# pengfeidip/pytorch-faster-rcnn

Measured on NVIDIA B200. Metric: images/sec of RPN proposal+assign+RoIAlign, R50-FPN 800x1333, higher is better.
Workload: dtype f32

## Files before the change

include/b200det.h:

```cpp
#ifndef B200DET_H_
#define B200DET_H_

#include <stddef.h>
#include <stdint.h>

#ifdef __cplusplus
extern "C" {
#endif

#if defined(__GNUC__)
#define B2D_API __attribute__((visibility("default")))
#else
#define B2D_API
#endif

#define B2D_OK 0
#define B2D_ERR_ARG (-1)
#define B2D_MAX_LEVELS 8
#define B2D_MAX_ANCHORS 16

typedef struct b2d_level {
    int H, W, A;
    int center_lt;
    float stride;
    float ws[B2D_MAX_ANCHORS], hs[B2D_MAX_ANCHORS];
    long long offset;
} b2d_level;

typedef struct b2d_pyramid {
    int num_levels;
    int _pad;
    long long total;
    b2d_level lv[B2D_MAX_LEVELS];
} b2d_pyramid;

B2D_API const char* b2d_last_error_string(void);
B2D_API int b2d_version(void);
B2D_API void b2d_reload_knobs(void);

B2D_API int b2d_anchor_grid(float* out, const float* ws, const float* hs, int A, int H, int W, float stride,
                    int center_lt, void* stream);
B2D_API int b2d_inside_anchor_mask(uint8_t* mask, const float* anchors, long long n, float img_h, float img_w,
                           float border, void* stream);
B2D_API int b2d_inside_grid_mask(float* flags, int A, int H, int W, int in_h, int in_w, void* stream);

B2D_API int b2d_calc_iou(float* out , const float* a , long long N, const float* b ,
                 long long K, void* stream);
B2D_API int b2d_elem_iou(float* out , const float* a, const float* b, long long N, void* stream);

B2D_API int b2d_assign_max_iou(int64_t* labels, float* max_iou, long long out_ld, const float* boxes,
                       long long box_ld, const int* box_count, long long N, const b2d_pyramid* pyr_host,
                       const float* img_hw, float border, const float* gt, int gt_ld, const int* gt_count,
                       int B, float pos_iou, float neg_iou, float min_pos_iou, int prepend_gt, int* census,
                       int* pos_list, int pos_cap, void* workspace, size_t ws_bytes, void* stream);

B2D_API int b2d_sample_labels(int* chosen, int* n_chosen, const int64_t* labels, long long ld, const int* count,
                      const int* count_add , long long n, const int* census, const int* pos_list, int pos_cap, int B, int max_num,
                      int pos_num, unsigned long long seed, const unsigned long long* seed_step , void* stream);
B2D_API int b2d_counter_add(unsigned long long* cell, unsigned long long inc, void* stream);
B2D_API int b2d_label_census(int* census, int* pos_list, int pos_cap, const int64_t* labels, long long ld,
                     const int* count, long long n, int B, void* stream);
B2D_API int b2d_scatter_sampled(int64_t* out, const int64_t* labels, long long ld, long long n, const int* chosen,
                        const int* n_chosen, int max_num, int B, void* stream);

B2D_API int b2d_bbox2param(float* out, const float* base, const float* bbox, long long n, const float* means_host,
                   const float* stds_host, void* stream);
B2D_API int b2d_param2bbox(float* out, const float* base, const float* param, long long n, const float* means_host,
                   const float* stds_host, int clamp, float img_h, float img_w, void* stream);
B2D_API int b2d_clamp_bbox(float* out, const float* bbox, long long n, float img_h, float img_w, void* stream);

B2D_API int b2d_encode_targets(float* tar_box, float* tar_gt, float* tar_param, int64_t* tar_label, int64_t* tar_is_gt,
                       const int* chosen, const int* n_chosen, int max_num, const int64_t* labels,
                       long long label_ld, const float* boxes, long long box_ld, const b2d_pyramid* pyr_host,
                       const float* gt, int gt_ld, const int* gt_count, const int64_t* gt_label,
                       int prepend_gt, const float* means_host, const float* stds_host, int B, void* stream);

B2D_API int b2d_roi_targets_fused(int64_t* labels, float* max_iou, long long out_ld, const float* boxes, long long box_ld,
                          const int* box_count, long long N, const float* gt, int gt_ld, const int* gt_count,
                          const int64_t* gt_label, int B, float pos_iou, float neg_iou, float min_pos_iou,
                          int prepend_gt, int* census, int* pos_list, int pos_cap, int* chosen, int* n_chosen,
                          int max_num, int pos_num, unsigned long long seed, const unsigned long long* seed_step,
                          float* tar_box, float* tar_gt, float* tar_param, int64_t* tar_label, int64_t* tar_is_gt,
                          const float* means_host, const float* stds_host, void* stream);

B2D_API int b2d_gather_head_outputs(float* tar_cls, float* tar_reg, const void* const* cls_ptrs_host,
                            const void* const* reg_ptrs_host, const b2d_pyramid* pyr_host, int cls_channels,
                            const int* chosen, const int* n_chosen, int max_num, int B, void* stream);

typedef struct b2d_rpn_cfg {
    int pre_nms, post_nms, max_num;
    int score_mode, num_cls_channels;
    float nms_thr_f;
    float min_size;
    float means[4], stds[4];
    int do_nms;
    float* records;
    void* event_after_select;
} b2d_rpn_cfg;

typedef struct b2d_roi_target_args {
    int64_t* labels; float* max_iou; long long out_ld;
    const float* gt; int gt_ld; const int* gt_count; const int64_t* gt_label;
    float pos_iou, neg_iou, min_pos_iou; int prepend_gt;
    int* census; int* pos_list; int pos_cap;
    int* chosen; int* n_chosen; int max_num, pos_num;
    unsigned long long seed; const unsigned long long* seed_step;
    float* tar_box; float* tar_gt; float* tar_param; int64_t* tar_label; int64_t* tar_is_gt;
    float means[4], stds[4];
} b2d_roi_target_args;

B2D_API size_t b2d_rpn_proposals_workspace_bytes(const b2d_pyramid* pyr_host, int B, const b2d_rpn_cfg* cfg_host);
B2D_API int b2d_last_launch_count(void);
B2D_API size_t b2d_rpn_proposals_debug_offset(const b2d_pyramid* pyr_host, int B, const b2d_rpn_cfg* cfg_host);
B2D_API int b2d_rpn_proposals(float* props, float* scores, int* count, int* prov, const void* const* cls_ptrs_host,
                      const void* const* reg_ptrs_host, const b2d_pyramid* pyr_host, const float* img_hw,
                      int B, const b2d_rpn_cfg* cfg_host, void* workspace, size_t ws_bytes, void* stream);

B2D_API int b2d_rpn_proposals_targets(float* props, float* scores, int* count, int* prov, const void* const* cls_ptrs_host,
                              const void* const* reg_ptrs_host, const b2d_pyramid* pyr_host, const float* img_hw,
                              int B, const b2d_rpn_cfg* cfg_host, void* workspace, size_t ws_bytes,
                              const b2d_roi_target_args* tg_host, void* stream);

B2D_API size_t b2d_topk_workspace_bytes(long long n_max, int S, int k);
B2D_API int b2d_topk(int* idx, int* out_count, const float* values, long long ld, const int* counts, long long n,
             int S, int k, void* workspace, size_t ws_bytes, void* stream);

B2D_API size_t b2d_nms_workspace_bytes(long long n_max, int S);
B2D_API int b2d_nms(int64_t* keep, int* keep_count, const float* boxes, const float* scores, long long n_ld,
            const int* counts, long long n, int S, float thr_f, int max_keep, int presorted, void* workspace,
            size_t ws_bytes, void* stream);

B2D_API size_t b2d_multiclass_nms_workspace_bytes(int cap);
B2D_API int b2d_multiclass_nms(float* out_box, float* out_score, int64_t* out_label, int* out_count, const float* bbox,
                       int box_classes, const float* score, long long n, int C, const unsigned long long* chan_mask_host,
                       float min_score, const float* score_factor, int strict, float nms_thr_f, int max_keep, int cap,
                       int* overflow, void* workspace, size_t ws_bytes, void* stream);
B2D_API int b2d_multiclass_candidates(float* cand_box, float* nms_box, float* cand_score, int* cand_label, int* cand_count,
                              int* overflow, const float* bbox, int box_classes, const float* score, long long n, int C,
                              const unsigned long long* chan_mask_host, float min_score, const float* score_factor,
                              int strict, int cap, void* stream);
B2D_API int b2d_batched_nms_boxes(float* out, const float* bbox, const int64_t* label, long long n, void* stream);
B2D_API int b2d_ga_pack_scores(float* out, long long ld, const void* const* cls_ptrs_host, const void* const* mask_ptrs_host,
                       const int* n_host, int L, void* stream);
B2D_API int b2d_ga_decode(float* box, float* score, int* nvalid, const int* idx, const float* packed, long long ld, int k,
                  const void* const* cls_ptrs_host, const void* const* mask_ptrs_host, const void* const* anchor_ptrs_host,
                  const void* const* reg_ptrs_host, const int* n_host, int L, const float* means_host, const float* stds_host,
                  float img_h, float img_w, float min_size, void* stream);
B2D_API int b2d_scale_rois(float* out, const float* rois, long long ld, long long n, float scale, void* stream);
B2D_API int b2d_iou_bin_ids(int* ids, const int64_t* labels, const float* iou, long long n, int num_bins,
                    const float* bin_lo_host, const float* bin_hi_host, void* stream);
B2D_API int b2d_sample_iou_balanced(int64_t* out_labels, const int64_t* labels, const float* iou, long long n, int max_num,
                            int pos_num, int num_bins, const float* bin_lo_host, const float* bin_hi_host,
                            unsigned long long seed, void* stream);
B2D_API size_t b2d_sampled_ce_workspace_bytes(void);
B2D_API int b2d_sampled_ce_fwd(float* partial, const float* logits, long long ld, int C, int row_major, int sigmoid,
                       const int64_t* target, long long rows, void* stream);
B2D_API int b2d_sampled_ce_bwd(float* grad, const float* scale, const float* logits, long long ld, int C, int row_major,
                       int sigmoid, const int64_t* target, long long rows, void* stream);

B2D_API size_t b2d_anchor_loss_workspace_bytes(const b2d_pyramid* pyr_host, int B);
B2D_API int b2d_anchor_loss_fwd(float* out3, const void* const* cls_ptrs_host, const void* const* reg_ptrs_host,
                        const b2d_pyramid* pyr_host, const int64_t* labels, long long label_ld, const float* gt, int gt_ld,
                        const int64_t* gt_label, int cls_channels, float alpha, float gamma, float beta,
                        const float* means_host, const float* stds_host, int B, void* workspace, size_t ws_bytes,
                        void* stream);
B2D_API int b2d_anchor_loss_bwd(void* const* dcls_ptrs_host, void* const* dreg_ptrs_host, const float* scale2,
                        const void* const* cls_ptrs_host, const void* const* reg_ptrs_host, const b2d_pyramid* pyr_host,
                        const int64_t* labels, long long label_ld, const float* gt, int gt_ld, const int64_t* gt_label,
                        int cls_channels, float alpha, float gamma, float beta, const float* means_host,
                        const float* stds_host, int B, void* stream);

B2D_API int b2d_fcos_targets(int64_t* cls_tar, float* reg_tar, float* ctr_tar, const b2d_pyramid* pyr_host, const float* gt,
                     int gt_ld, const int* gt_count, const int64_t* gt_label, const float* img_hw,
                     const float* level_thr_host, int B, void* stream);

B2D_API size_t b2d_rcnn_detect_workspace_bytes(int cap, int B);
B2D_API int b2d_rcnn_detect(float* out_box, float* out_score, int64_t* out_label, int* out_count, const float* props,
                    long long ld, const int* counts, long long n, const float* cls_out, const float* reg_out, int C,
                    int reg_classes, const float* means_host, const float* stds_host, const float* img_hw,
                    float min_score, float nms_thr_f, int max_per_img, int strict, int cap, int B, int* overflow,
                    void* workspace, size_t ws_bytes, void* stream);
B2D_API int b2d_rcnn_detect_records(float* out_box, float* out_score, int64_t* out_label, int* out_count, float* records,
                            const float* props, long long ld, const int* counts, long long n, const float* cls_out,
                            const float* reg_out, int C, int reg_classes, const float* means_host, const float* stds_host,
                            const float* img_hw, float min_score, float nms_thr_f, int max_per_img, int strict, int cap,
                            int B, int* overflow, void* workspace, size_t ws_bytes, void* stream);

typedef struct b2d_dense_levels {
    int num_levels, _pad;
    long long offset[B2D_MAX_LEVELS];
    const float* base[B2D_MAX_LEVELS];
    long long img_stride[B2D_MAX_LEVELS], class_stride[B2D_MAX_LEVELS];
} b2d_dense_levels;
B2D_API int b2d_dense_detect(float* out_box, float* out_score, int64_t* out_label, int* out_count, const float* boxes,
                     long long ld, const int* counts, const int* rows, const b2d_dense_levels* lv_host, int C, int transform,
                     const float* score_factor, long long factor_ld, const unsigned long long* chan_mask_host,
                     float min_score, int label_add, float nms_thr_f, int max_per_img, int strict, int cap, int B,
                     int* overflow, void* workspace, size_t ws_bytes, void* const* events_host, void* stream);
B2D_API int b2d_dense_detect_records(float* out_box, float* out_score, int64_t* out_label, int* out_count, float* records,
                             const float* boxes, long long ld, const int* counts, const int* rows,
                             const b2d_dense_levels* lv_host, int C, int transform, const float* score_factor,
                             long long factor_ld, const unsigned long long* chan_mask_host, float min_score, int label_add,
                             float nms_thr_f, int max_per_img, int strict, int cap, int B, int* overflow, void* workspace,
                             size_t ws_bytes, void* const* events_host, void* stream);

typedef struct b2d_roi_cfg {
    int num_levels, C, PH, PW, sampling_ratio, aligned, layout;
    float finest_scale;
    int H[B2D_MAX_LEVELS], W[B2D_MAX_LEVELS];
    float spatial_scale[B2D_MAX_LEVELS];
} b2d_roi_cfg;

B2D_API int b2d_roi_align_fwd(float* out, const void* const* feat_ptrs_host, const float* rois, long long roi_ld,
                      const int* roi_img, const int* levels, long long R, const b2d_roi_cfg* cfg_host,
                      void* stream);
B2D_API int b2d_roi_align_fwd_batched(float* out, const void* const* feat_ptrs_host, const float* rois, long long ld,
                              const int* counts, int B, const b2d_roi_cfg* cfg_host, void* stream);
B2D_API size_t b2d_roi_align_bwd_workspace_bytes(long long R, int B, const b2d_roi_cfg* cfg_host);
B2D_API int b2d_roi_align_bwd(void* const* grad_feat_ptrs_host, const float* grad_out, const float* rois,
                      long long roi_ld, const int* roi_img, const int* levels, long long R, int B,
                      const b2d_roi_cfg* cfg_host, void* workspace, size_t ws_bytes, void* stream);
B2D_API int b2d_nchw_to_nhwc(float* dst, const float* src, int B, int C, int H, int W, void* stream);
B2D_API int b2d_roi_levels(int* levels, const float* rois, long long roi_ld, long long R, float finest_scale,
                   int num_levels, void* stream);

B2D_API size_t b2d_roi_cell_bitmap_bytes(int B, const b2d_roi_cfg* cfg_host);
B2D_API int b2d_roi_mark_cells(void* bitmap, const float* rois, long long ld, const int* counts, int B,
                       const b2d_roi_cfg* cfg_host, void* stream);
B2D_API int b2d_fetch_marked_cells(void* const* dst_ptrs_host, const void* const* src_ptrs_host, const void* bitmap,
                           int B, const b2d_roi_cfg* cfg_host, unsigned long long* moved_cells, void* stream);

B2D_API int b2d_roi_pool_fwd(float* out, int* argmax, const float* feat, int B, int C, int H, int W, const float* rois,
                     long long roi_ld, const int* roi_img, long long R, float spatial_scale, int PH, int PW,
                     void* stream);
B2D_API int b2d_roi_pool_bwd(float* grad_feat, const float* grad_out, const int* argmax, int B, int C, int H, int W,
                     const float* rois, long long roi_ld, const int* roi_img, long long R, float spatial_scale,
                     int PH, int PW, void* workspace, size_t ws_bytes, void* stream);

B2D_API int b2d_refine_bboxes(float* out, int* out_count, const float* props, long long ld, const int* counts,
                      long long n, const int64_t* label, const float* reg_out, int C, const int64_t* is_gt,
                      const float* means_host, const float* stds_host, int clamp, const float* img_hw, int B,
                      void* stream);
B2D_API int b2d_refine_bboxes_argmax(float* out, int* out_count, const float* props, long long ld, const int* counts,
                             long long n, const float* cls_out, int num_classes, const float* reg_out,
                             int reg_classes, const float* means_host, const float* stds_host, const float* img_hw,
                             int B, void* stream);

B2D_API size_t b2d_atss_workspace_bytes(const b2d_pyramid* pyr_host, int B);
B2D_API int b2d_atss_assign(int64_t* cls_tar, float* reg_tar, float* ctr_tar, const b2d_pyramid* pyr_host,
                    const float* gt, int gt_ld, const int* gt_count, const int64_t* gt_label, const float* img_hw,
                    int B, int topk, void* workspace, size_t ws_bytes, void* stream);

B2D_API int b2d_fcos_decode(float* boxes, float* key, float* score, float* ctr_score, const void* const* cls_ptrs_host,
                    const void* const* reg_ptrs_host, const void* const* ctr_ptrs_host, const b2d_pyramid* pyr_host,
                    int cls_channels, float reg_mean, float reg_std, float min_size, const float* img_hw, int B,
                    void* stream);
B2D_API size_t b2d_dense_select_workspace_bytes(const int* level_sizes_host, int num_levels, int B, int pre_nms);
B2D_API int b2d_dense_select(int* idx, int* count, float* sel_boxes, const float* key, const float* boxes,
                     const int* level_sizes_host, int num_levels, int B, int pre_nms, void* workspace, size_t ws_bytes,
                     void* stream);

#ifdef __cplusplus
}
#endif
#endif
```

pytorch-faster-rcnn_b200/_C.py:

```python
import ctypes
import os

import numpy as np
import torch

_HERE = os.path.dirname(os.path.abspath(__file__))
LIB_PATH = os.path.join(_HERE, "libb200det.so")

MAX_LEVELS = 8
MAX_ANCHORS = 16

c_void_p, c_int, c_ll, c_float, c_size_t, c_ull = (ctypes.c_void_p, ctypes.c_int, ctypes.c_longlong,
                                                   ctypes.c_float, ctypes.c_size_t, ctypes.c_ulonglong)


class Level(ctypes.Structure):
    _fields_ = [("H", c_int), ("W", c_int), ("A", c_int), ("center_lt", c_int), ("stride", c_float),
                ("ws", c_float * MAX_ANCHORS), ("hs", c_float * MAX_ANCHORS), ("offset", c_ll)]


class Pyramid(ctypes.Structure):
    _fields_ = [("num_levels", c_int), ("_pad", c_int), ("total", c_ll), ("lv", Level * MAX_LEVELS)]


class RpnCfg(ctypes.Structure):
    _fields_ = [("pre_nms", c_int), ("post_nms", c_int), ("max_num", c_int), ("score_mode", c_int),
                ("num_cls_channels", c_int), ("nms_thr_f", c_float), ("min_size", c_float),
                ("means", c_float * 4), ("stds", c_float * 4), ("do_nms", c_int), ("records", c_void_p), ("event_after_select", c_void_p)]


class RoiTargetArgs(ctypes.Structure):
    _fields_ = [("labels", c_void_p), ("max_iou", c_void_p), ("out_ld", c_ll), ("gt", c_void_p), ("gt_ld", c_int),
                ("gt_count", c_void_p), ("gt_label", c_void_p), ("pos_iou", c_float), ("neg_iou", c_float),
                ("min_pos_iou", c_float), ("prepend_gt", c_int), ("census", c_void_p), ("pos_list", c_void_p),
                ("pos_cap", c_int), ("chosen", c_void_p), ("n_chosen", c_void_p), ("max_num", c_int), ("pos_num", c_int),
                ("seed", c_ull), ("seed_step", c_void_p), ("tar_box", c_void_p), ("tar_gt", c_void_p),
                ("tar_param", c_void_p), ("tar_label", c_void_p), ("tar_is_gt", c_void_p), ("means", c_float * 4),
                ("stds", c_float * 4)]


class RoiCfg(ctypes.Structure):
    _fields_ = [("num_levels", c_int), ("C", c_int), ("PH", c_int), ("PW", c_int), ("sampling_ratio", c_int),
                ("aligned", c_int), ("layout", c_int), ("finest_scale", c_float), ("H", c_int * MAX_LEVELS),
                ("W", c_int * MAX_LEVELS), ("spatial_scale", c_float * MAX_LEVELS)]


class DenseLevels(ctypes.Structure):
    _fields_ = [("num_levels", c_int), ("_pad", c_int), ("offset", c_ll * MAX_LEVELS), ("base", c_void_p * MAX_LEVELS),
                ("img_stride", c_ll * MAX_LEVELS), ("class_stride", c_ll * MAX_LEVELS)]


class B200DetError(RuntimeError):
    pass


_lib = None

_P = c_void_p
_SIGS = {
    "b2d_anchor_grid": [_P, _P, _P, c_int, c_int, c_int, c_float, c_int, _P],
    "b2d_inside_anchor_mask": [_P, _P, c_ll, c_float, c_float, c_float, _P],
    "b2d_inside_grid_mask": [_P, c_int, c_int, c_int, c_int, c_int, _P],
    "b2d_calc_iou": [_P, _P, c_ll, _P, c_ll, _P],
    "b2d_elem_iou": [_P, _P, _P, c_ll, _P],
    "b2d_assign_max_iou": [_P, _P, c_ll, _P, c_ll, _P, c_ll, _P, _P, c_float, _P, c_int, _P, c_int, c_float,
                           c_float, c_float, c_int, _P, _P, c_int, _P, c_size_t, _P],
    "b2d_sample_labels": [_P, _P, _P, c_ll, _P, _P, c_ll, _P, _P, c_int, c_int, c_int, c_int, c_ull, _P, _P],
    "b2d_counter_add": [_P, c_ull, _P],
    "b2d_roi_targets_fused": [_P, _P, c_ll, _P, c_ll, _P, c_ll, _P, c_int, _P, _P, c_int, c_float, c_float, c_float,
                              c_int, _P, _P, c_int, _P, _P, c_int, c_int, c_ull, _P, _P, _P, _P, _P, _P, _P, _P, _P],
    "b2d_anchor_loss_fwd": [_P, _P, _P, _P, _P, c_ll, _P, c_int, _P, c_int, c_float, c_float, c_float, _P, _P, c_int, _P,
                            c_size_t, _P],
    "b2d_anchor_loss_bwd": [_P, _P, _P, _P, _P, _P, _P, c_ll, _P, c_int, _P, c_int, c_float, c_float, c_float, _P, _P,
                            c_int, _P],
    "b2d_fcos_targets": [_P, _P, _P, _P, _P, c_int, _P, _P, _P, _P, c_int, _P],
    "b2d_rcnn_detect": [_P, _P, _P, _P, _P, c_ll, _P, c_ll, _P, _P, c_int, c_int, _P, _P, _P, c_float, c_float, c_int,
                        c_int, c_int, c_int, _P, _P, c_size_t, _P],
    "b2d_rcnn_detect_records": [_P, _P, _P, _P, _P, _P, c_ll, _P, c_ll, _P, _P, c_int, c_int, _P, _P, _P, c_float, c_float,
                                c_int, c_int, c_int, c_int, _P, _P, c_size_t, _P],
    "b2d_dense_detect": [_P, _P, _P, _P, _P, c_ll, _P, _P, _P, c_int, c_int, _P, c_ll, _P, c_float, c_int, c_float, c_int,
                         c_int, c_int, c_int, _P, _P, c_size_t, _P, _P],
    "b2d_dense_detect_records": [_P, _P, _P, _P, _P, _P, c_ll, _P, _P, _P, c_int, c_int, _P, c_ll, _P, c_float, c_int, c_float,
                                 c_int, c_int, c_int, c_int, _P, _P, c_size_t, _P, _P],
    "b2d_dense_select": [_P, _P, _P, _P, _P, _P, c_int, c_int, c_int, _P, c_size_t, _P],
    "b2d_gather_head_outputs": [_P, _P, _P, _P, _P, c_int, _P, _P, c_int, c_int, _P],
    "b2d_roi_align_fwd_batched": [_P, _P, _P, c_ll, _P, c_int, _P, _P],
    "b2d_label_census": [_P, _P, c_int, _P, c_ll, _P, c_ll, c_int, _P],
    "b2d_scatter_sampled": [_P, _P, c_ll, c_ll, _P, _P, c_int, c_int, _P],
    "b2d_bbox2param": [_P, _P, _P, c_ll, _P, _P, _P],
    "b2d_param2bbox": [_P, _P, _P, c_ll, _P, _P, c_int, c_float, c_float, _P],
    "b2d_clamp_bbox": [_P, _P, c_ll, c_float, c_float, _P],
    "b2d_encode_targets": [_P, _P, _P, _P, _P, _P, _P, c_int, _P, c_ll, _P, c_ll, _P, _P, c_int, _P, _P, c_int,
                           _P, _P, c_int, _P],
    "b2d_rpn_proposals": [_P, _P, _P, _P, _P, _P, _P, _P, c_int, _P, _P, c_size_t, _P],
    "b2d_rpn_proposals_targets": [_P, _P, _P, _P, _P, _P, _P, _P, c_int, _P, _P, c_size_t, _P, _P],
    "b2d_topk": [_P, _P, _P, c_ll, _P, c_ll, c_int, c_int, _P, c_size_t, _P],
    "b2d_nms": [_P, _P, _P, _P, c_ll, _P, c_ll, c_int, c_float, c_int, c_int, _P, c_size_t, _P],
    "b2d_roi_align_fwd": [_P, _P, _P, c_ll, _P, _P, c_ll, _P, _P],
    "b2d_roi_align_bwd": [_P, _P, _P, c_ll, _P, _P, c_ll, c_int, _P, _P, c_size_t, _P],
    "b2d_roi_levels": [_P, _P, c_ll, c_ll, c_float, c_int, _P],
    "b2d_nchw_to_nhwc": [_P, _P, c_int, c_int, c_int, c_int, _P],
    "b2d_refine_bboxes": [_P, _P, _P, c_ll, _P, c_ll, _P, _P, c_int, _P, _P, _P, c_int, _P, c_int, _P],
    "b2d_refine_bboxes_argmax": [_P, _P, _P, c_ll, _P, c_ll, _P, c_int, _P, c_int, _P, _P, _P, c_int, _P],
    "b2d_atss_assign": [_P, _P, _P, _P, _P, c_int, _P, _P, _P, c_int, c_int, _P, c_size_t, _P],
    "b2d_fcos_decode": [_P, _P, _P, _P, _P, _P, _P, _P, c_int, c_float, c_float, c_float, _P, c_int, _P],
    "b2d_roi_pool_fwd": [_P, _P, _P, c_int, c_int, c_int, c_int, _P, c_ll, _P, c_ll, c_float, c_int, c_int, _P],
    "b2d_multiclass_nms": [_P, _P, _P, _P, _P, c_int, _P, c_ll, c_int, _P, c_float, _P, c_int, c_float, c_int, c_int, _P, _P,
                           c_size_t, _P],
    "b2d_multiclass_candidates": [_P, _P, _P, _P, _P, _P, _P, c_int, _P, c_ll, c_int, _P, c_float, _P, c_int, c_int, _P],
    "b2d_batched_nms_boxes": [_P, _P, _P, c_ll, _P],
    "b2d_scale_rois": [_P, _P, c_ll, c_ll, c_float, _P],
    "b2d_iou_bin_ids": [_P, _P, _P, c_ll, c_int, _P, _P, _P],
    "b2d_sample_iou_balanced": [_P, _P, _P, c_ll, c_int, c_int, c_int, _P, _P, c_ull, _P],
    "b2d_sampled_ce_fwd": [_P, _P, c_ll, c_int, c_int, c_int, _P, c_ll, _P],
    "b2d_sampled_ce_bwd": [_P, _P, _P, c_ll, c_int, c_int, c_int, _P, c_ll, _P],
    "b2d_ga_pack_scores": [_P, c_ll, _P, _P, _P, c_int, _P],
    "b2d_ga_decode": [_P, _P, _P, _P, _P, c_ll, c_int, _P, _P, _P, _P, _P, c_int, _P, _P, c_float, c_float, c_float, _P],
    "b2d_roi_mark_cells": [_P, _P, c_ll, _P, c_int, _P, _P],
    "b2d_fetch_marked_cells": [_P, _P, _P, c_int, _P, _P, _P],
    "b2d_roi_pool_bwd": [_P, _P, _P, c_int, c_int, c_int, c_int, _P, c_ll, _P, c_ll, c_float, c_int, c_int, _P,
                         c_size_t, _P],
}
_SIZE_FNS = {
    "b2d_rpn_proposals_workspace_bytes": [_P, c_int, _P],
    "b2d_rpn_proposals_debug_offset": [_P, c_int, _P],
    "b2d_topk_workspace_bytes": [c_ll, c_int, c_int],
    "b2d_nms_workspace_bytes": [c_ll, c_int],
    "b2d_roi_align_bwd_workspace_bytes": [c_ll, c_int, _P],
    "b2d_atss_workspace_bytes": [_P, c_int],
    "b2d_rcnn_detect_workspace_bytes": [c_int, c_int],
    "b2d_dense_select_workspace_bytes": [_P, c_int, c_int, c_int],
    "b2d_anchor_loss_workspace_bytes": [_P, c_int],
    "b2d_multiclass_nms_workspace_bytes": [c_int],
    "b2d_sampled_ce_workspace_bytes": [],
    "b2d_roi_cell_bitmap_bytes": [c_int, _P],
}
EXPORTS = sorted(list(_SIGS) + list(_SIZE_FNS) + ["b2d_last_error_string", "b2d_version", "b2d_reload_knobs", "b2d_last_launch_count"])


def lib():
    global _lib
    if _lib is not None:
        return _lib
    if not os.path.exists(LIB_PATH):
        raise B200DetError(
            "libb200det.so is not built (%s). Run `python __graft_entry__.py build` "
            "(nvcc, sm_100a). There is no CPU or PyTorch fallback." % LIB_PATH)
    L = ctypes.CDLL(LIB_PATH)
    for name, sig in _SIGS.items():
        fn = getattr(L, name)
        fn.argtypes = sig
        fn.restype = c_int
    for name, sig in _SIZE_FNS.items():
        fn = getattr(L, name)
        fn.argtypes = sig
        fn.restype = c_size_t
    L.b2d_last_error_string.restype = ctypes.c_char_p
    L.b2d_version.restype = c_int
    L.b2d_reload_knobs.restype = None
    L.b2d_last_launch_count.restype = c_int
    _lib = L
    return L


def reload_knobs():
    lib().b2d_reload_knobs()


def check(rc, what):
    if rc != 0:
        msg = lib().b2d_last_error_string().decode("utf-8", "replace")
        raise B200DetError("%s failed (rc=%d): %s" % (what, rc, msg))


def call(name, *args):
    check(getattr(lib(), name)(*args), name)


def ptr(t):
    if t is None:
        return None
    return c_void_p(t.data_ptr())


def stream():
    return c_void_p(torch.cuda.current_stream().cuda_stream)


def require_cuda(*tensors):
    for t in tensors:
        if t is not None and not t.is_cuda:
            raise B200DetError("b200det kernels need CUDA tensors (got a %s tensor); there is no CPU fallback"
                               % t.device.type)


def f32c(t):
    if t.dtype != torch.float32:
        t = t.to(torch.float32)
    return t.contiguous()


def host_f4(v, default):
    a = np.asarray(default if v is None else v, dtype=np.float32).reshape(-1)
    if a.size != 4:
        raise ValueError("expected 4 values, got %r" % (v,))
    return (c_float * 4)(*a.tolist())


def floor_f32(x):
    f = np.float32(x)
    if float(f) > float(x):
        f = np.nextafter(f, np.float32(-np.inf), dtype=np.float32)
    return float(f)


def make_pyramid(levels):
    if not 1 <= len(levels) <= MAX_LEVELS:
        raise ValueError("1..%d levels supported" % MAX_LEVELS)
    p = Pyramid()
    p.num_levels = len(levels)
    off = 0
    for i, lv in enumerate(levels):
        A = len(lv["ws"])
        if not 1 <= A <= MAX_ANCHORS:
            raise ValueError("1..%d anchors per cell supported" % MAX_ANCHORS)
        L = p.lv[i]
        L.H, L.W, L.A = int(lv["H"]), int(lv["W"]), A
        L.center_lt = int(bool(lv.get("center_lt", False)))
        L.stride = float(lv["stride"])
        for a in range(A):
            L.ws[a] = float(lv["ws"][a])
            L.hs[a] = float(lv["hs"][a])
        L.offset = off
        off += A * L.H * L.W
    p.total = off
    return p
```

pytorch-faster-rcnn_b200/csrc/assign.cu:

```cuda
#include <cstdlib>
#include <cstring>

#include "common.cuh"
#include "targets_common.cuh"

namespace b2d {

__device__ __forceinline__ void grid_limits(const b2d_level& lv, float img_h, float img_w, int& in_h, int& in_w) {
    const double r = 1.0 / (double)lv.stride;
    in_h = min(lv.H, (int)((double)img_h * r) + 1);
    in_w = min(lv.W, (int)((double)img_w * r) + 1);
}

__device__ __forceinline__ bool load_box(const AssignArgs& p, const b2d_pyramid& pyr, int b, long long i,
                                         long long n_b, Box& bx, const int* __restrict__ s_lim) {
    if (i >= n_b) return false;
    if (!p.use_pyr) {
        const float* src = p.boxes + (long long)b * 4 * p.box_ld;
        bx.x1 = src[i]; bx.y1 = src[p.box_ld + i]; bx.x2 = src[2 * p.box_ld + i]; bx.y2 = src[3 * p.box_ld + i];
        return true;
    }
    int l = 0;
#pragma unroll
    for (int q = 1; q < kMaxLevels; ++q)
        if (q < pyr.num_levels && i >= pyr.lv[q].offset) l = q;
    const b2d_level& lv = pyr.lv[l];
    const int li = (int)(i - lv.offset);
    const int hw = lv.H * lv.W;
    const int a = li / hw, r = li - a * hw;
    const int y = r / lv.W, x = r - y * lv.W;
    bx = anchor_at(lv, a, y, x);
    const float img_h = p.img_hw[2 * b], img_w = p.img_hw[2 * b + 1];
    bool ok = (y < s_lim[2 * l]) && (x < s_lim[2 * l + 1]);
    if (p.border >= 0.0f)
        ok = ok && bx.x1 >= -p.border && bx.y1 >= -p.border && bx.x2 < img_w + p.border && bx.y2 < img_h + p.border;
    return ok;
}

__global__ void __launch_bounds__(256) k_assign_colmax(AssignArgs p, b2d_pyramid pyr, uint32_t* __restrict__ colmax) {
    __shared__ Box s_gt[kGtChunk];
    __shared__ float s_ga[kGtChunk];
    __shared__ uint32_t s_max[kGtChunk];
    const int b = blockIdx.y;
    const int K = p.gt_count[b];
    const long long n_b = p.box_count ? (long long)p.box_count[b] : p.N;
    const float* g = p.gt + (long long)b * 4 * p.gt_ld;
    const uint32_t kNegInf = f2key(-INFINITY), kZero = f2key(0.0f);
    __shared__ int s_lim[2 * kMaxLevels];
    if (p.use_pyr && threadIdx.x < pyr.num_levels)
        grid_limits(pyr.lv[threadIdx.x], p.img_hw[2 * b], p.img_hw[2 * b + 1], s_lim[2 * threadIdx.x], s_lim[2 * threadIdx.x + 1]);
    __syncthreads();

    Box bx[kBoxesPerThread];
    float ba[kBoxesPerThread];
    bool ok[kBoxesPerThread];
    const long long base = ((long long)blockIdx.x * blockDim.x) * kBoxesPerThread + threadIdx.x;
#pragma unroll
    for (int r = 0; r < kBoxesPerThread; ++r) {
        ok[r] = load_box(p, pyr, b, base + (long long)r * blockDim.x, n_b, bx[r], s_lim);
        ba[r] = ok[r] ? area_plus1(bx[r]) : 0.0f;
    }
    bool any_ok = false;
#pragma unroll
    for (int r = 0; r < kBoxesPerThread; ++r) any_ok |= ok[r];
    any_ok = __any_sync(0xffffffffu, any_ok);
    for (int j0 = 0; j0 < K; j0 += kGtChunk) {
        const int kc = min(kGtChunk, K - j0);
        __syncthreads();
        for (int j = threadIdx.x; j < kc; j += blockDim.x) {
            Box t{g[j0 + j], g[p.gt_ld + j0 + j], g[2 * p.gt_ld + j0 + j], g[3 * p.gt_ld + j0 + j]};
            s_gt[j] = t; s_ga[j] = area_plus1(t); s_max[j] = kNegInf;
        }
        __syncthreads();
        for (int j = 0; j < kc; ++j) {
            const Box t = s_gt[j];
            const float ta = s_ga[j];
            uint32_t m = any_ok ? kZero : kNegInf;
#pragma unroll
            for (int r = 0; r < kBoxesPerThread; ++r) {
                if (!ok[r]) continue;
                const bool hit = fmaxf(bx[r].x1, t.x1) < fminf(bx[r].x2, t.x2) && fmaxf(bx[r].y1, t.y1) < fminf(bx[r].y2, t.y2);
                if (hit || !(ba[r] > 0.0f && ta > 0.0f)) {
                    const float v = iou_plus1(bx[r], ba[r], t, ta) + 0.0f;
                    m = max(m, f2key(v));
                }
            }
            if (__any_sync(0xffffffffu, m > kZero) || j0 + j == 0 || !any_ok) {
                m = __reduce_max_sync(0xffffffffu, m);
                if (lane_id() == 0 && m > s_max[j]) atomicMax(&s_max[j], m);
            } else if (lane_id() == 0 && s_max[j] < kZero) {
                atomicMax(&s_max[j], kZero);
            }
        }
        __syncthreads();
        for (int j = threadIdx.x; j < kc; j += blockDim.x)
            if (s_max[j] != kNegInf) atomicMax(&colmax[(long long)b * p.gt_ld + j0 + j], s_max[j]);
    }
}

__global__ void __launch_bounds__(256) k_assign_label(AssignArgs p, b2d_pyramid pyr,
                                                      const uint32_t* __restrict__ colmax,
                                                      int64_t* __restrict__ labels, float* __restrict__ out_iou,
                                                      int* __restrict__ census, int* __restrict__ pos_list,
                                                      int pos_cap) {
    __shared__ Box s_gt[kGtChunk];
    __shared__ float s_ga[kGtChunk];
    __shared__ float s_cm[kGtChunk];
    __shared__ int s_cnt[2];
    const int b = blockIdx.y;
    const int K = p.gt_count[b];
    const long long n_b = p.box_count ? (long long)p.box_count[b] : p.N;
    const float* g = p.gt + (long long)b * 4 * p.gt_ld;
    const int lead = p.prepend_gt ? K : 0;
    if (threadIdx.x < 2) s_cnt[threadIdx.x] = 0;
    __shared__ int s_lim[2 * kMaxLevels];
    if (p.use_pyr && threadIdx.x < pyr.num_levels)
        grid_limits(pyr.lv[threadIdx.x], p.img_hw[2 * b], p.img_hw[2 * b + 1], s_lim[2 * threadIdx.x], s_lim[2 * threadIdx.x + 1]);
    __syncthreads();

    Box bx[kBoxesPerThread];
    float ba[kBoxesPerThread], best[kBoxesPerThread], veq[kBoxesPerThread];
    int arg[kBoxesPerThread], eq[kBoxesPerThread];
    bool ok[kBoxesPerThread];
    const long long base = ((long long)blockIdx.x * blockDim.x) * kBoxesPerThread + threadIdx.x;
#pragma unroll
    for (int r = 0; r < kBoxesPerThread; ++r) {
        ok[r] = load_box(p, pyr, b, base + (long long)r * blockDim.x, n_b, bx[r], s_lim);
        ba[r] = ok[r] ? area_plus1(bx[r]) : 0.0f;
        best[r] = 0.0f; veq[r] = 0.0f; arg[r] = 0; eq[r] = -1;
    }
    for (int j0 = 0; j0 < K; j0 += kGtChunk) {
        const int kc = min(kGtChunk, K - j0);
        __syncthreads();
        for (int j = threadIdx.x; j < kc; j += blockDim.x) {
            Box t{g[j0 + j], g[p.gt_ld + j0 + j], g[2 * p.gt_ld + j0 + j], g[3 * p.gt_ld + j0 + j]};
            s_gt[j] = t; s_ga[j] = area_plus1(t);
            s_cm[j] = key2f(colmax[(long long)b * p.gt_ld + j0 + j]);
        }
        __syncthreads();
        for (int j = 0; j < kc; ++j) {
            const Box t = s_gt[j];
            const float ta = s_ga[j], cm = s_cm[j];
            const bool cm_ok = cm >= p.min_pos_iou;
            const bool need_all = (j0 + j) == 0 || (cm_ok && cm == 0.0f) || !(ta > 0.0f);
#pragma unroll
            for (int r = 0; r < kBoxesPerThread; ++r) {
                if (!ok[r]) continue;
                const bool hit = fmaxf(bx[r].x1, t.x1) < fminf(bx[r].x2, t.x2) && fmaxf(bx[r].y1, t.y1) < fminf(bx[r].y2, t.y2);
                if (!(hit || need_all || !(ba[r] > 0.0f))) continue;
                const float v = iou_plus1(bx[r], ba[r], t, ta);
                if ((j0 + j) == 0 || v > best[r]) { best[r] = v; arg[r] = j0 + j; }
                if (eq[r] < 0 && cm_ok && v == cm) { eq[r] = j0 + j; veq[r] = v; }
            }
        }
    }
    int64_t* lab = labels + (long long)b * p.out_ld;
    float* oiou = out_iou + (long long)b * p.out_ld;
    int* plist = pos_list ? pos_list + (long long)b * pos_cap : nullptr;
#pragma unroll
    for (int r = 0; r < kBoxesPerThread; ++r) {
        const long long i = base + (long long)r * blockDim.x;
        int64_t out_l = -1;
        float out_v = 0.0f;
        const bool in_range = i < n_b;
        if (ok[r]) {
            int l = -1;
            if (best[r] < p.neg_iou) l = 0;
            if (best[r] >= p.pos_iou) l = 1;
            int a = arg[r];
            out_v = best[r];
            if (eq[r] >= 0) { l = 1; a = eq[r]; out_v = veq[r]; }
            out_l = (l == 1) ? (int64_t)(a + 1) : (int64_t)l;
        }
        if (in_range) { lab[lead + i] = out_l; oiou[lead + i] = out_v; }
        const bool is_pos = in_range && out_l > 0, is_neg = in_range && out_l == 0;
        const unsigned mp = __ballot_sync(0xffffffffu, is_pos), mn = __ballot_sync(0xffffffffu, is_neg);
        if (lane_id() == 0) {
            if (mp) atomicAdd(&s_cnt[0], __popc(mp));
            if (mn) atomicAdd(&s_cnt[1], __popc(mn));
        }
        if (plist) {
            const int slot = warp_alloc(is_pos, &census[4 * b + 2]);
            if (is_pos && slot < pos_cap) plist[slot] = (int)(lead + i);
        }
    }
    if (p.prepend_gt && blockIdx.x == 0) {
        for (int j = threadIdx.x; j < K; j += blockDim.x) {
            lab[j] = j + 1; oiou[j] = 1.0f;
            if (plist) { const int slot = atomicAdd(&census[4 * b + 2], 1); if (slot < pos_cap) plist[slot] = j; }
        }
        if (threadIdx.x == 0) atomicAdd(&s_cnt[0], K);
    }
    __syncthreads();
    if (threadIdx.x < 2 && s_cnt[threadIdx.x]) atomicAdd(&census[4 * b + threadIdx.x], s_cnt[threadIdx.x]);
}


constexpr int kRowAnchors = 4;

__device__ __forceinline__ bool anchor_valid(const AssignArgs& p, const Box& a, int y, int x, int in_h, int in_w,
                                             float img_h, float img_w) {
    bool ok = (y < in_h) && (x < in_w);
    if (p.border >= 0.0f)
        ok = ok && a.x1 >= -p.border && a.y1 >= -p.border && a.x2 < img_w + p.border && a.y2 < img_h + p.border;
    return ok;
}

constexpr int kRectChunks = 4;

__global__ void __launch_bounds__(256) k_colmax_rect(AssignArgs p, b2d_pyramid pyr, uint32_t* __restrict__ colmax,
                                                     int max_a) {
    __shared__ uint32_t s_red[8];
    const int b = blockIdx.y;
    int w = blockIdx.x;
    const int rc = w % kRectChunks; w /= kRectChunks;
    const int a = w % max_a; w /= max_a;
    const int l = w % pyr.num_levels;
    const int j = w / pyr.num_levels;
    if (j >= p.gt_count[b]) return;
    const b2d_level& lv = pyr.lv[l];
    if (a >= lv.A) return;
    const float* g = p.gt + (long long)b * 4 * p.gt_ld;
    const Box t{g[j], g[p.gt_ld + j], g[2 * p.gt_ld + j], g[3 * p.gt_ld + j]};
    const float ta = area_plus1(t);
    const float img_h = p.img_hw[2 * b], img_w = p.img_hw[2 * b + 1];
    int in_h, in_w;
    grid_limits(lv, img_h, img_w, in_h, in_w);
    const float s = lv.stride;
    const float hw = lv.ws[a] / 2.0f, hh = lv.hs[a] / 2.0f, off = lv.center_lt ? 0.0f : s / 2.0f;
    int x0 = 0, x1 = lv.W - 1, y0 = 0, y1 = lv.H - 1;
    if (ta > 0.0f) {
        x0 = max(0, (int)floorf((t.x1 - hw - off) / s) - 1);
        x1 = min(lv.W - 1, (int)ceilf((t.x2 + hw - off) / s) + 1);
        y0 = max(0, (int)floorf((t.y1 - hh - off) / s) - 1);
        y1 = min(lv.H - 1, (int)ceilf((t.y2 + hh - off) / s) + 1);
    }
    const int rw = x1 - x0 + 1;
    uint32_t m = 0u;
    if (rw > 0) {
        const int tx = threadIdx.x % 64, ty = threadIdx.x / 64;
        for (int y = y0 + rc + ty * kRectChunks; y <= y1; y += 4 * kRectChunks) {
            for (int x = x0 + tx; x <= x1; x += 64) {
                const Box an = anchor_at(lv, a, y, x);
                if (!anchor_valid(p, an, y, x, in_h, in_w, img_h, img_w)) continue;
                m = max(m, f2key(iou_plus1(an, area_plus1(an), t, ta) + 0.0f));
            }
        }
    }
    m = __reduce_max_sync(0xffffffffu, m);
    if (lane_id() == 0) s_red[threadIdx.x >> 5] = m;
    __syncthreads();
    if (threadIdx.x == 0) {
        for (int q = 1; q < 8; ++q) m = max(m, s_red[q]);
        if (m) atomicMax(&colmax[(long long)b * p.gt_ld + j], m);
    }
}

__global__ void __launch_bounds__(256) k_label_rows(AssignArgs p, b2d_pyramid pyr, const uint32_t* __restrict__ colmax,
                                                    int64_t* __restrict__ labels, float* __restrict__ out_iou,
                                                    int* __restrict__ census, int* __restrict__ pos_list, int pos_cap) {
    __shared__ Box s_gt[kGtChunk];
    __shared__ float s_ga[kGtChunk];
    __shared__ float s_cm[kGtChunk];
    __shared__ unsigned char s_all[kGtChunk];
    __shared__ int s_cnt[2];
    const int b = blockIdx.y;
    const int K = p.gt_count[b];
    const float* g = p.gt + (long long)b * 4 * p.gt_ld;
    const float img_h = p.img_hw[2 * b], img_w = p.img_hw[2 * b + 1];
    if (threadIdx.x < 2) s_cnt[threadIdx.x] = 0;
    const long long i0 = ((long long)blockIdx.x * blockDim.x + threadIdx.x) * kRowAnchors;
    Box bx[kRowAnchors];
    float ba[kRowAnchors], best[kRowAnchors], veq[kRowAnchors];
    int arg[kRowAnchors], eq[kRowAnchors];
    bool ok[kRowAnchors], live[kRowAnchors];
    float ylo = INFINITY, yhi = -INFINITY;
    {
        int l = -1, a = 0, y = 0, x = 0, in_h = 0, in_w = 0;
        long long lend = -1;
#pragma unroll
        for (int q = 0; q < kRowAnchors; ++q) {
            const long long i = i0 + q;
            live[q] = i < pyr.total;
            ok[q] = false;
            bx[q] = Box{0.f, 0.f, 0.f, 0.f};
            if (live[q]) {
                if (i >= lend) {
                    l = 0;
                    for (int r = 1; r < pyr.num_levels; ++r) if (i >= pyr.lv[r].offset) l = r;
                    const b2d_level& nv = pyr.lv[l];
                    const int li = (int)(i - nv.offset), hw = nv.H * nv.W;
                    a = li / hw;
                    const int r2 = li - a * hw;
                    y = r2 / nv.W; x = r2 - y * nv.W;
                    lend = nv.offset + (long long)nv.A * hw;
                    grid_limits(nv, img_h, img_w, in_h, in_w);
                }
                const b2d_level& lv = pyr.lv[l];
                bx[q] = anchor_at(lv, a, y, x);
                ok[q] = anchor_valid(p, bx[q], y, x, in_h, in_w, img_h, img_w);
                if (++x == lv.W) { x = 0; if (++y == lv.H) { y = 0; ++a; } }
            }
            ba[q] = ok[q] ? area_plus1(bx[q]) : 0.0f;
            if (ok[q]) { ylo = fminf(ylo, bx[q].y1); yhi = fmaxf(yhi, bx[q].y2); }
            best[q] = 0.0f; veq[q] = 0.0f; arg[q] = 0; eq[q] = -1;
        }
    }
    for (int j0 = 0; j0 < K; j0 += kGtChunk) {
        const int kc = min(kGtChunk, K - j0);
        __syncthreads();
        for (int j = threadIdx.x; j < kc; j += blockDim.x) {
            Box t{g[j0 + j], g[p.gt_ld + j0 + j], g[2 * p.gt_ld + j0 + j], g[3 * p.gt_ld + j0 + j]};
            const float ta = area_plus1(t);
            const uint32_t ck = colmax[(long long)b * p.gt_ld + j0 + j];
            const float cm = ck ? fmaxf(key2f(ck), 0.0f) : 0.0f;
            s_gt[j] = t; s_ga[j] = ta; s_cm[j] = cm;
            s_all[j] = ((j0 + j) == 0 || (cm >= p.min_pos_iou && cm == 0.0f) || !(ta > 0.0f)) ? 1 : 0;
        }
        __syncthreads();
        for (int j = 0; j < kc; ++j) {
            const Box t = s_gt[j];
            const bool all = s_all[j] != 0;
            if (!all && !(fmaxf(ylo, t.y1) < fminf(yhi, t.y2))) continue;
            const float ta = s_ga[j], cm = s_cm[j];
            const bool cm_ok = cm >= p.min_pos_iou;
#pragma unroll
            for (int q = 0; q < kRowAnchors; ++q) {
                if (!ok[q]) continue;
                const bool hit = fmaxf(bx[q].x1, t.x1) < fminf(bx[q].x2, t.x2) && fmaxf(bx[q].y1, t.y1) < fminf(bx[q].y2, t.y2);
                if (!(hit || all || !(ba[q] > 0.0f))) continue;
                const float v = iou_plus1(bx[q], ba[q], t, ta);
                if ((j0 + j) == 0 || v > best[q]) { best[q] = v; arg[q] = j0 + j; }
                if (eq[q] < 0 && cm_ok && v == cm) { eq[q] = j0 + j; veq[q] = v; }
            }
        }
    }
    int64_t* lab = labels + (long long)b * p.out_ld;
    float* oiou = out_iou + (long long)b * p.out_ld;
    int* plist = pos_list ? pos_list + (long long)b * pos_cap : nullptr;
    int64_t ol[kRowAnchors];
    float ov[kRowAnchors];
#pragma unroll
    for (int q = 0; q < kRowAnchors; ++q) {
        ol[q] = -1; ov[q] = 0.0f;
        if (ok[q]) {
            int lb = -1;
            if (best[q] < p.neg_iou) lb = 0;
            if (best[q] >= p.pos_iou) lb = 1;
            int a = arg[q];
            ov[q] = best[q];
            if (eq[q] >= 0) { lb = 1; a = eq[q]; ov[q] = veq[q]; }
            ol[q] = (lb == 1) ? (int64_t)(a + 1) : (int64_t)lb;
        }
    }
    const bool vec = live[kRowAnchors - 1] && ((reinterpret_cast<uintptr_t>(lab) & 15) == 0) &&
                     ((reinterpret_cast<uintptr_t>(oiou) & 15) == 0);
    if (vec) {
        reinterpret_cast<longlong2*>(lab + i0)[0] = make_longlong2(ol[0], ol[1]);
        reinterpret_cast<longlong2*>(lab + i0)[1] = make_longlong2(ol[2], ol[3]);
        *reinterpret_cast<float4*>(oiou + i0) = make_float4(ov[0], ov[1], ov[2], ov[3]);
    } else {
#pragma unroll
        for (int q = 0; q < kRowAnchors; ++q)
            if (live[q]) { lab[i0 + q] = ol[q]; oiou[i0 + q] = ov[q]; }
    }
#pragma unroll
    for (int q = 0; q < kRowAnchors; ++q) {
        const bool is_pos = live[q] && ol[q] > 0, is_neg = live[q] && ol[q] == 0;
        const unsigned mp = __ballot_sync(0xffffffffu, is_pos), mn = __ballot_sync(0xffffffffu, is_neg);
        if (lane_id() == 0) {
            if (mp) atomicAdd(&s_cnt[0], __popc(mp));
            if (mn) atomicAdd(&s_cnt[1], __popc(mn));
        }
        if (plist) {
            const int slot = warp_alloc(is_pos, &census[4 * b + 2]);
            if (is_pos && slot < pos_cap) plist[slot] = (int)(i0 + q);
        }
    }
    __syncthreads();
    if (threadIdx.x < 2 && s_cnt[threadIdx.x]) atomicAdd(&census[4 * b + threadIdx.x], s_cnt[threadIdx.x]);
}

__device__ __forceinline__ void assign_small_body(const AssignArgs& p, SmallSmem& sm, int64_t* __restrict__ labels,
                                                  float* __restrict__ out_iou, int* __restrict__ census,
                                                  int* __restrict__ pos_list, int pos_cap, int* s_lab) {
    Box* s_gt = sm.gt;
    float* s_ga = sm.ga;
    uint32_t* s_max = sm.mx;
    int* s_cnt = sm.cnt;
    const int b = blockIdx.x;
    const int K = p.gt_count[b];
    const int n_b = p.box_count ? p.box_count[b] : (int)p.N;
    const float* g = p.gt + (long long)b * 4 * p.gt_ld;
    const float* src = p.boxes + (long long)b * 4 * p.box_ld;
    const int lead = p.prepend_gt ? K : 0;
    const uint32_t kNegInf = f2key(-INFINITY);
    if (threadIdx.x < 3) s_cnt[threadIdx.x] = 0;
    for (int j = threadIdx.x; j < K; j += blockDim.x) {
        Box t{g[j], g[p.gt_ld + j], g[2 * p.gt_ld + j], g[3 * p.gt_ld + j]};
        s_gt[j] = t; s_ga[j] = area_plus1(t); s_max[j] = kNegInf;
    }
    Box bx[kSmallBoxes];
    float ba[kSmallBoxes];
    bool ok[kSmallBoxes];
#pragma unroll
    for (int r = 0; r < kSmallBoxes; ++r) {
        const int i = threadIdx.x + r * kSmallThreads;
        ok[r] = i < n_b;
        if (ok[r]) bx[r] = Box{src[i], src[p.box_ld + i], src[2 * p.box_ld + i], src[3 * p.box_ld + i]};
        else bx[r] = Box{0.f, 0.f, 0.f, 0.f};
        ba[r] = ok[r] ? area_plus1(bx[r]) : 0.0f;
    }
    __syncthreads();
    for (int j = 0; j < K; ++j) {
        const Box t = s_gt[j];
        const float ta = s_ga[j];
        uint32_t m = kNegInf;
#pragma unroll
        for (int r = 0; r < kSmallBoxes; ++r)
            if (ok[r]) m = max(m, f2key(iou_plus1(bx[r], ba[r], t, ta) + 0.0f));
        m = __reduce_max_sync(0xffffffffu, m);
        if (lane_id() == 0 && m != kNegInf) atomicMax(&s_max[j], m);
    }
    __syncthreads();
    float best[kSmallBoxes], veq[kSmallBoxes];
    int arg[kSmallBoxes], eq[kSmallBoxes];
#pragma unroll
    for (int r = 0; r < kSmallBoxes; ++r) { best[r] = 0.0f; veq[r] = 0.0f; arg[r] = 0; eq[r] = -1; }
    for (int j = 0; j < K; ++j) {
        const Box t = s_gt[j];
        const float ta = s_ga[j], cm = key2f(s_max[j]);
        const bool cm_ok = cm >= p.min_pos_iou;
#pragma unroll
        for (int r = 0; r < kSmallBoxes; ++r) {
            if (!ok[r]) continue;
            const float v = iou_plus1(bx[r], ba[r], t, ta);
            if (j == 0 || v > best[r]) { best[r] = v; arg[r] = j; }
            if (eq[r] < 0 && cm_ok && v == cm) { eq[r] = j; veq[r] = v; }
        }
    }
    int64_t* lab = labels + (long long)b * p.out_ld;
    float* oiou = out_iou + (long long)b * p.out_ld;
    int* plist = pos_list ? pos_list + (long long)b * pos_cap : nullptr;
#pragma unroll
    for (int r = 0; r < kSmallBoxes; ++r) {
        const int i = threadIdx.x + r * kSmallThreads;
        int64_t out_l = -1;
        float out_v = 0.0f;
        if (ok[r]) {
            int l = -1;
            if (best[r] < p.neg_iou) l = 0;
            if (best[r] >= p.pos_iou) l = 1;
            int a = arg[r];
            out_v = best[r];
            if (eq[r] >= 0) { l = 1; a = eq[r]; out_v = veq[r]; }
            out_l = (l == 1) ? (int64_t)(a + 1) : (int64_t)l;
            lab[lead + i] = out_l; oiou[lead + i] = out_v;
            if (s_lab) s_lab[lead + i] = (int)out_l;
        }
        const bool is_pos = ok[r] && out_l > 0, is_neg = ok[r] && out_l == 0;
        const unsigned mp = __ballot_sync(0xffffffffu, is_pos), mn = __ballot_sync(0xffffffffu, is_neg);
        if (lane_id() == 0) {
            if (mp) atomicAdd(&s_cnt[0], __popc(mp));
            if (mn) atomicAdd(&s_cnt[1], __popc(mn));
        }
        if (plist) {
            const int slot = warp_alloc(is_pos, &s_cnt[2]);
            if (is_pos && slot < pos_cap) plist[slot] = lead + i;
        }
    }
    __syncthreads();
    if (p.prepend_gt) {
        for (int j = threadIdx.x; j < K; j += blockDim.x) {
            lab[j] = j + 1; oiou[j] = 1.0f;
            if (s_lab) s_lab[j] = j + 1;
            if (plist) { const int slot = atomicAdd(&s_cnt[2], 1); if (slot < pos_cap) plist[slot] = j; }
        }
        __syncthreads();
    }
    if (threadIdx.x == 0) {
        census[4 * b + 0] = s_cnt[0] + (p.prepend_gt ? K : 0);
        census[4 * b + 1] = s_cnt[1];
        census[4 * b + 2] = s_cnt[2];
        census[4 * b + 3] = 0;
    }
    __syncthreads();
}

__global__ void __launch_bounds__(kSmallThreads) k_assign_small(AssignArgs p, int64_t* __restrict__ labels,
                                                                float* __restrict__ out_iou, int* __restrict__ census,
                                                                int* __restrict__ pos_list, int pos_cap) {
    __shared__ SmallSmem sm;
    assign_small_body(p, sm, labels, out_iou, census, pos_list, pos_cap, nullptr);
}

__global__ void __launch_bounds__(256) k_label_census(int* __restrict__ census, int* __restrict__ pos_list,
                                                      int pos_cap, const int64_t* __restrict__ labels,
                                                      long long ld, const int* __restrict__ count, long long n) {
    __shared__ int s_cnt[2];
    const int b = blockIdx.y;
    if (threadIdx.x < 2) s_cnt[threadIdx.x] = 0;
    __syncthreads();
    const long long n_b = count ? (long long)count[b] : n;
    const long long i = (long long)blockIdx.x * blockDim.x + threadIdx.x;
    const int64_t l = (i < n_b) ? labels[(long long)b * ld + i] : -1;
    const bool is_pos = l > 0, is_neg = (i < n_b) && l == 0;
    const unsigned mp = __ballot_sync(0xffffffffu, is_pos), mn = __ballot_sync(0xffffffffu, is_neg);
    if (lane_id() == 0) {
        if (mp) atomicAdd(&s_cnt[0], __popc(mp));
        if (mn) atomicAdd(&s_cnt[1], __popc(mn));
    }
    if (pos_list) {
        const int slot = warp_alloc(is_pos, &census[4 * b + 2]);
        if (is_pos && slot < pos_cap) pos_list[(long long)b * pos_cap + slot] = (int)i;
    }
    __syncthreads();
    if (threadIdx.x < 2 && s_cnt[threadIdx.x]) atomicAdd(&census[4 * b + threadIdx.x], s_cnt[threadIdx.x]);
}

constexpr int kSampleThreads = 1024;
constexpr int kSampleSortCap = 4096;

__global__ void __launch_bounds__(kSampleThreads) k_sample(int* __restrict__ chosen, int* __restrict__ n_chosen,
                                                           const int64_t* __restrict__ labels, long long ld,
                                                           const int* __restrict__ count,
                                                           const int* __restrict__ count_add, long long n,
                                                           const int* __restrict__ census,
                                                           const int* __restrict__ pos_list, int pos_cap,
                                                           int max_num, int pos_num, unsigned long long seed,
                                                           const unsigned long long* __restrict__ seed_step) {
    extern __shared__ __align__(16) uint64_t s_sort[];
    if (seed_step) seed += *seed_step;
    __shared__ int s_n, s_warp[kSampleThreads / 32], s_take;
    __shared__ unsigned long long s_lo, s_hi;
    const int b = blockIdx.x;
    const int64_t* lab = labels + (long long)b * ld;
    const long long n_b = (count ? (long long)count[b] : n) + (count_add ? (long long)count_add[b] : 0);
    const int npos = min(census[4 * b + 0], pos_cap);
    const int nneg = census[4 * b + 1];
    const int* plist = pos_list + (long long)b * pos_cap;
    const uint64_t sd = seed + 0x632BE59BD9B4E019ull * (uint64_t)(b + 1);
    int* out = chosen + (long long)b * max_num;
    if (threadIdx.x == 0) s_n = 0;
    __syncthreads();

    const int keep_pos = min(npos, pos_num);
    uint64_t thr = ~0ull;
    if (npos > pos_num) {
        if (threadIdx.x == 0) { s_lo = 0ull; s_hi = ~0ull; }
        __syncthreads();
        for (int it = 0; it < 64; ++it) {
            const unsigned long long lo = s_lo, hi = s_hi;
            if (lo >= hi) break;
            const unsigned long long mid = lo + (hi - lo) / 2;
            int c = 0;
            for (int t = threadIdx.x; t < npos; t += blockDim.x) {
                const uint32_t idx = (uint32_t)plist[t];
                const uint64_t comp = ((uint64_t)mix_key(sd, idx) << 32) | idx;
                c += (comp <= mid);
            }
            c = __reduce_add_sync(0xffffffffu, c);
            if (lane_id() == 0) s_warp[threadIdx.x >> 5] = c;
            __syncthreads();
            if (threadIdx.x == 0) {
                int tot = 0;
                for (int w = 0; w < (int)(blockDim.x >> 5); ++w) tot += s_warp[w];
                if (tot >= pos_num) s_hi = mid; else s_lo = mid + 1;
            }
            __syncthreads();
        }
        thr = s_lo;
    }
    for (int t0 = 0; t0 < npos; t0 += blockDim.x) {
        const int t = t0 + threadIdx.x;
        bool take = false;
        uint32_t idx = 0;
        if (t < npos) {
            idx = (uint32_t)plist[t];
            take = (((uint64_t)mix_key(sd, idx) << 32) | idx) <= thr;
        }
        const int slot = warp_alloc(take, &s_n);
        if (take && slot < kSampleSortCap) s_sort[slot] = (uint64_t)idx;
    }
    __syncthreads();
    const int want_neg = min(max(max_num - keep_pos, 0), nneg);
    if (want_neg > 0) {
        int bits = 2;
        while ((1ll << bits) < n_b) ++bits;
        if (bits & 1) ++bits;
        const int half = bits >> 1;
        const long long dom = 1ll << bits;
        if (threadIdx.x == 0) s_take = 0;
        __syncthreads();
        if (blockDim.x <= 256) {
            __shared__ int s_cnt4[4][8];
            const int nw = blockDim.x >> 5, wq = threadIdx.x >> 5;
            for (long long t0 = 0; t0 < dom; t0 += 4ll * blockDim.x) {
                uint32_t y[4];
                bool hit[4];
                unsigned m[4];
#pragma unroll
                for (int q = 0; q < 4; ++q) {
                    const long long t = t0 + (long long)q * blockDim.x + threadIdx.x;
                    y[q] = feistel((uint32_t)t, half, sd ^ 0xA5A5A5A5DEADBEEFull);
                    hit[q] = t < dom && ((long long)y[q] < n_b) && (lab[y[q]] == 0);
                }
#pragma unroll
                for (int q = 0; q < 4; ++q) {
                    m[q] = __ballot_sync(0xffffffffu, hit[q]);
                    if (lane_id() == 0) s_cnt4[q][wq] = __popc(m[q]);
                }
                __syncthreads();
                int before = s_take, tot = 0;
#pragma unroll
                for (int q = 0; q < 4; ++q) {
                    int mine = before + tot;
                    for (int w = 0; w < nw; ++w) { if (w < wq) mine += s_cnt4[q][w]; tot += s_cnt4[q][w]; }
                    const int rank = mine + __popc(m[q] & ((1u << lane_id()) - 1u));
                    if (hit[q] && rank < want_neg) s_sort[keep_pos + rank] = (uint64_t)y[q];
                }
                __syncthreads();
                if (threadIdx.x == 0) s_take += tot;
                __syncthreads();
                if (s_take >= want_neg) break;
            }
        } else
        for (long long t0 = 0; t0 < dom; t0 += blockDim.x) {
            const uint32_t y = feistel((uint32_t)(t0 + threadIdx.x), half, sd ^ 0xA5A5A5A5DEADBEEFull);
            const bool hit = ((long long)y < n_b) && (lab[y] == 0);
            const unsigned m = __ballot_sync(0xffffffffu, hit);
            if (lane_id() == 0) s_warp[threadIdx.x >> 5] = __popc(m);
            __syncthreads();
            int before = s_take;
            for (int w = 0; w < (threadIdx.x >> 5); ++w) before += s_warp[w];
            const int rank = before + __popc(m & ((1u << lane_id()) - 1u));
            if (hit && rank < want_neg) s_sort[keep_pos + rank] = (uint64_t)y;
            __syncthreads();
            if (threadIdx.x == 0) {
                int tot = 0;
                for (int w = 0; w < (int)(blockDim.x >> 5); ++w) tot += s_warp[w];
                s_take += tot;
            }
            __syncthreads();
            if (s_take >= want_neg) break;
        }
    }
    __syncthreads();
    const int total = keep_pos + want_neg;
    int p2 = 1;
    while (p2 < total) p2 <<= 1;
    for (int t = threadIdx.x; t < p2; t += blockDim.x)
        s_sort[t] = (t < total) ? (0xffffffffull - s_sort[t]) + 1ull : 0ull;
    __syncthreads();
    bitonic_sort_desc(s_sort, p2);
    for (int t = threadIdx.x; t < max_num; t += blockDim.x)
        out[t] = (t < total) ? (int)(0xffffffffull - (s_sort[t] - 1ull)) : -1;
    if (threadIdx.x == 0) n_chosen[b] = total;
}

__global__ void __launch_bounds__(256) k_scatter_sampled(int64_t* __restrict__ out, const int64_t* __restrict__ labels,
                                                         long long ld, const int* __restrict__ chosen,
                                                         const int* __restrict__ n_chosen, int max_num) {
    const int b = blockIdx.y;
    const int t = blockIdx.x * blockDim.x + threadIdx.x;
    if (t >= n_chosen[b]) return;
    const int i = chosen[(long long)b * max_num + t];
    out[(long long)b * ld + i] = labels[(long long)b * ld + i];
}

struct EncArgs {
    const int* chosen; const int* n_chosen; int max_num;
    const int64_t* labels; long long label_ld;
    const float* boxes; long long box_ld; int use_pyr;
    const float* gt; int gt_ld; const int* gt_count; const int64_t* gt_label;
    int prepend_gt;
    float ms[8];
};

__global__ void __launch_bounds__(128) k_encode_targets(EncArgs p, b2d_pyramid pyr, float* __restrict__ tar_box,
                                                        float* __restrict__ tar_gt, float* __restrict__ tar_param,
                                                        int64_t* __restrict__ tar_label,
                                                        int64_t* __restrict__ tar_is_gt) {
    const int b = blockIdx.y;
    const int t = blockIdx.x * blockDim.x + threadIdx.x;
    if (t >= p.max_num) return;
    const long long o = (long long)b * 4 * p.max_num;
    const bool live = t < p.n_chosen[b];
    Box bx{0, 0, 0, 0}, gb{0, 0, 0, 0};
    float prm[4] = {0, 0, 0, 0};
    int64_t lab_out = 0, isgt = 0;
    if (live) {
        const int K = p.gt_count[b];
        const int lead = p.prepend_gt ? K : 0;
        const int i = p.chosen[(long long)b * p.max_num + t];
        const int64_t lab = p.labels[(long long)b * p.label_ld + i];
        const float* g = p.gt + (long long)b * 4 * p.gt_ld;
        if (i < lead) {
            bx = Box{g[i], g[p.gt_ld + i], g[2 * p.gt_ld + i], g[3 * p.gt_ld + i]};
            isgt = 1;
        } else if (p.use_pyr) {
            const long long ii = i - lead;
            int l = 0;
            for (int q = 1; q < pyr.num_levels; ++q)
                if (ii >= pyr.lv[q].offset) l = q;
            bx = anchor_flat(pyr.lv[l], (int)(ii - pyr.lv[l].offset));
        } else {
            const float* src = p.boxes + (long long)b * 4 * p.box_ld;
            const long long ii = i - lead;
            bx = Box{src[ii], src[p.box_ld + ii], src[2 * p.box_ld + ii], src[3 * p.box_ld + ii]};
        }
        const int j = (int)max(lab - 1, (int64_t)0);
        gb = Box{g[j], g[p.gt_ld + j], g[2 * p.gt_ld + j], g[3 * p.gt_ld + j]};
        const float bw = (bx.x2 - bx.x1) + 1.0f, bh = (bx.y2 - bx.y1) + 1.0f;
        const float gw = (gb.x2 - gb.x1) + 1.0f, gh = (gb.y2 - gb.y1) + 1.0f;
        const float bcx = (bx.x2 + bx.x1) / 2.0f, bcy = (bx.y2 + bx.y1) / 2.0f;
        const float gcx = (gb.x2 + gb.x1) / 2.0f, gcy = (gb.y2 + gb.y1) / 2.0f;
        prm[0] = ((gcx - bcx) / bw - p.ms[0]) / p.ms[4];
        prm[1] = ((gcy - bcy) / bh - p.ms[1]) / p.ms[5];
        prm[2] = (logf(gw / bw) - p.ms[2]) / p.ms[6];
        prm[3] = (logf(gh / bh) - p.ms[3]) / p.ms[7];
        if (p.gt_label) lab_out = (lab > 0) ? p.gt_label[(long long)b * p.gt_ld + j] : 0;
        else lab_out = (lab > 0) ? 1 : 0;
    }
    if (tar_box) { tar_box[o + t] = bx.x1; tar_box[o + p.max_num + t] = bx.y1; tar_box[o + 2 * p.max_num + t] = bx.x2; tar_box[o + 3 * p.max_num + t] = bx.y2; }
    if (tar_gt) { tar_gt[o + t] = gb.x1; tar_gt[o + p.max_num + t] = gb.y1; tar_gt[o + 2 * p.max_num + t] = gb.x2; tar_gt[o + 3 * p.max_num + t] = gb.y2; }
    if (tar_param) { tar_param[o + t] = prm[0]; tar_param[o + p.max_num + t] = prm[1]; tar_param[o + 2 * p.max_num + t] = prm[2]; tar_param[o + 3 * p.max_num + t] = prm[3]; }
    if (tar_label) tar_label[(long long)b * p.max_num + t] = lab_out;
    if (tar_is_gt) tar_is_gt[(long long)b * p.max_num + t] = isgt;
}

struct GatherArgs {
    const float* cls[kMaxLevels]; const float* reg[kMaxLevels];
    const int* chosen; const int* n_chosen; int max_num, cls_ch;
};

__global__ void __launch_bounds__(128) k_gather_head(GatherArgs p, b2d_pyramid pyr, float* __restrict__ tar_cls,
                                                     float* __restrict__ tar_reg) {
    const int b = blockIdx.y;
    const int t = blockIdx.x * blockDim.x + threadIdx.x;
    if (t >= p.max_num) return;
    const bool live = t < p.n_chosen[b];
    int l = 0, li = 0;
    long long n = 1;
    if (live) {
        const int i = p.chosen[(long long)b * p.max_num + t];
        for (int q = 1; q < pyr.num_levels; ++q) if (i >= pyr.lv[q].offset) l = q;
        li = (int)(i - pyr.lv[l].offset);
        n = (long long)pyr.lv[l].A * pyr.lv[l].H * pyr.lv[l].W;
    }
    for (int c = 0; c < p.cls_ch; ++c)
        tar_cls[((long long)b * p.cls_ch + c) * p.max_num + t] = live ? p.cls[l][((long long)b * p.cls_ch + c) * n + li] : 0.0f;
    for (int c = 0; c < 4; ++c)
        tar_reg[((long long)b * 4 + c) * p.max_num + t] = live ? p.reg[l][((long long)b * 4 + c) * n + li] : 0.0f;
}

__global__ void __launch_bounds__(kSmallThreads) k_roi_targets_small(AssignArgs p, int64_t* __restrict__ labels,
                                                                     float* __restrict__ out_iou,
                                                                     int* __restrict__ census, int* __restrict__ pos_list,
                                                                     int pos_cap, FusedArgs f) {
    __shared__ SmallSmem sm;
    __shared__ FusedScratch fs;
    pdl_wait();
    assign_small_body(p, sm, labels, out_iou, census, pos_list, pos_cap, fs.lab);
    fused_sample_encode(p, f, sm.gt, fs, sm.cnt[0], sm.cnt[1], blockIdx.x);
}

__global__ void k_counter_add(unsigned long long* cell, unsigned long long inc) { *cell += inc; }

__global__ void k_fill_u32(uint32_t* p, uint32_t v, long long n) {
    const long long i = (long long)blockIdx.x * blockDim.x + threadIdx.x;
    if (i < n) p[i] = v;
}

}

using namespace b2d;

extern "C" {

int b2d_assign_max_iou(int64_t* labels, float* max_iou, long long out_ld, const float* boxes, long long box_ld,
                       const int* box_count, long long N, const b2d_pyramid* pyr_host, const float* img_hw,
                       float border, const float* gt, int gt_ld, const int* gt_count, int B, float pos_iou,
                       float neg_iou, float min_pos_iou, int prepend_gt, int* census, int* pos_list, int pos_cap,
                       void* workspace, size_t ws_bytes, void* stream) {
    B2D_REQUIRE(labels && max_iou && gt && gt_count && census, "assign_max_iou: null pointer");
    B2D_REQUIRE(boxes || (pyr_host && img_hw), "assign_max_iou: need boxes or pyramid+img_hw");
    B2D_REQUIRE(B >= 1 && gt_ld >= 1 && N >= 0, "assign_max_iou: bad sizes");
    B2D_REQUIRE(workspace && ws_bytes >= (size_t)B * gt_ld * 4, "assign_max_iou: workspace too small");
    cudaStream_t st = (cudaStream_t)stream;
    AssignArgs a;
    a.boxes = boxes; a.box_ld = box_ld; a.box_count = box_count; a.N = N;
    a.use_pyr = boxes ? 0 : 1; a.img_hw = img_hw; a.border = border;
    a.gt = gt; a.gt_ld = gt_ld; a.gt_count = gt_count;
    a.pos_iou = pos_iou; a.neg_iou = neg_iou; a.min_pos_iou = min_pos_iou;
    a.prepend_gt = prepend_gt; a.out_ld = out_ld;
    b2d_pyramid pyr;
    memset(&pyr, 0, sizeof(pyr));
    if (a.use_pyr) { pyr = *pyr_host; a.N = pyr.total; }
    if (!a.use_pyr && N <= kSmallThreads * kSmallBoxes && gt_ld <= kGtChunk) {
        k_assign_small<<<B, kSmallThreads, 0, st>>>(a, labels, max_iou, census, pos_list, pos_cap);
        return check_launch("assign_max_iou");
    }
    if (a.use_pyr && !prepend_gt && !knobs().assign_old) {
        uint32_t* cmx = (uint32_t*)workspace;
        cudaMemsetAsync(census, 0, sizeof(int) * 4 * B, st);
        cudaMemsetAsync(cmx, 0, sizeof(uint32_t) * (size_t)B * gt_ld, st);
        int max_a = 1;
        for (int l = 0; l < pyr.num_levels; ++l) max_a = max(max_a, pyr.lv[l].A);
        dim3 g1(gt_ld * pyr.num_levels * max_a * kRectChunks, B);
        k_colmax_rect<<<g1, 256, 0, st>>>(a, pyr, cmx, max_a);
        dim3 g2(cdiv(pyr.total, 256 * kRowAnchors), B);
        k_label_rows<<<g2, 256, 0, st>>>(a, pyr, cmx, labels, max_iou, census, pos_list, pos_cap);
        return check_launch("assign_max_iou");
    }
    uint32_t* colmax = (uint32_t*)workspace;
    const long long nc = (long long)B * gt_ld;
    k_fill_u32<<<cdiv(nc, 256), 256, 0, st>>>(colmax, f2key(-INFINITY), nc);
    cudaMemsetAsync(census, 0, sizeof(int) * 4 * B, st);
    const int per_block = 256 * kBoxesPerThread;
    dim3 grid(cdiv(a.N > 0 ? a.N : 1, per_block), B);
    k_assign_colmax<<<grid, 256, 0, st>>>(a, pyr, colmax);
    k_assign_label<<<grid, 256, 0, st>>>(a, pyr, colmax, labels, max_iou, census, pos_list, pos_cap);
    return check_launch("assign_max_iou");
}

int b2d_label_census(int* census, int* pos_list, int pos_cap, const int64_t* labels, long long ld,
                     const int* count, long long n, int B, void* stream) {
    B2D_REQUIRE(census && labels && B >= 1 && n >= 0, "label_census: bad args");
    cudaStream_t st = (cudaStream_t)stream;
    cudaMemsetAsync(census, 0, sizeof(int) * 4 * B, st);
    if (n == 0) return B2D_OK;
    dim3 grid(cdiv(n, 256), B);
    k_label_census<<<grid, 256, 0, st>>>(census, pos_list, pos_cap, labels, ld, count, n);
    return check_launch("label_census");
}

int b2d_sample_labels(int* chosen, int* n_chosen, const int64_t* labels, long long ld, const int* count,
                      const int* count_add, long long n, const int* census, const int* pos_list, int pos_cap, int B, int max_num,
                      int pos_num, unsigned long long seed, const unsigned long long* seed_step, void* stream) {
    B2D_REQUIRE(chosen && n_chosen && labels && census && pos_list, "sample_labels: null pointer");
    B2D_REQUIRE(B >= 1 && max_num >= 1 && max_num <= kSampleSortCap && pos_num >= 0 && pos_num <= max_num,
                "sample_labels: need 1 <= max_num <= 4096 and pos_num <= max_num");
    B2D_REQUIRE(n < (1ll << 31), "sample_labels: n too large");
    B2D_SMEM(k_sample, kSampleSortCap * 8, "k_sample");
    const int threads = (knobs().sample_threads == 128 || knobs().sample_threads == 256) ? knobs().sample_threads : kSampleThreads;
    k_sample<<<B, threads, kSampleSortCap * 8, (cudaStream_t)stream>>>(
        chosen, n_chosen, labels, ld, count, count_add, n, census, pos_list, pos_cap, max_num, pos_num, seed, seed_step);
    return check_launch("sample_labels");
}

int b2d_counter_add(unsigned long long* cell, unsigned long long inc, void* stream) {
    B2D_REQUIRE(cell, "counter_add: null pointer");
    k_counter_add<<<1, 1, 0, (cudaStream_t)stream>>>(cell, inc);
    return check_launch("counter_add");
}

int b2d_scatter_sampled(int64_t* out, const int64_t* labels, long long ld, long long n, const int* chosen,
                        const int* n_chosen, int max_num, int B, void* stream) {
    B2D_REQUIRE(out && labels && chosen && n_chosen && B >= 1, "scatter_sampled: bad args");
    (void)n;
    dim3 grid(cdiv(max_num, 256), B);
    k_scatter_sampled<<<grid, 256, 0, (cudaStream_t)stream>>>(out, labels, ld, chosen, n_chosen, max_num);
    return check_launch("scatter_sampled");
}

int b2d_gather_head_outputs(float* tar_cls, float* tar_reg, const void* const* cls_ptrs_host,
                            const void* const* reg_ptrs_host, const b2d_pyramid* pyr_host, int cls_channels,
                            const int* chosen, const int* n_chosen, int max_num, int B, void* stream) {
    B2D_REQUIRE(tar_cls && tar_reg && cls_ptrs_host && reg_ptrs_host && pyr_host && chosen && n_chosen,
                "gather_head_outputs: null pointer");
    GatherArgs p;
    memset(&p, 0, sizeof(p));
    for (int l = 0; l < pyr_host->num_levels; ++l) { p.cls[l] = (const float*)cls_ptrs_host[l]; p.reg[l] = (const float*)reg_ptrs_host[l]; }
    p.chosen = chosen; p.n_chosen = n_chosen; p.max_num = max_num; p.cls_ch = cls_channels;
    dim3 grid(cdiv(max_num, 128), B);
    k_gather_head<<<grid, 128, 0, (cudaStream_t)stream>>>(p, *pyr_host, tar_cls, tar_reg);
    return check_launch("gather_head_outputs");
}

int b2d_encode_targets(float* tar_box, float* tar_gt, float* tar_param, int64_t* tar_label, int64_t* tar_is_gt,
                       const int* chosen, const int* n_chosen, int max_num, const int64_t* labels,
                       long long label_ld, const float* boxes, long long box_ld, const b2d_pyramid* pyr_host,
                       const float* gt, int gt_ld, const int* gt_count, const int64_t* gt_label, int prepend_gt,
                       const float* means_host, const float* stds_host, int B, void* stream) {
    B2D_REQUIRE(chosen && n_chosen && labels && gt && gt_count, "encode_targets: null pointer");
    B2D_REQUIRE(boxes || pyr_host, "encode_targets: need boxes or pyramid");
    EncArgs p;
    p.chosen = chosen; p.n_chosen = n_chosen; p.max_num = max_num; p.labels = labels; p.label_ld = label_ld;
    p.boxes = boxes; p.box_ld = box_ld; p.use_pyr = boxes ? 0 : 1;
    p.gt = gt; p.gt_ld = gt_ld; p.gt_count = gt_count; p.gt_label = gt_label; p.prepend_gt = prepend_gt;
    for (int i = 0; i < 4; ++i) { p.ms[i] = means_host ? means_host[i] : 0.0f; p.ms[4 + i] = stds_host ? stds_host[i] : 1.0f; }
    b2d_pyramid pyr;
    memset(&pyr, 0, sizeof(pyr));
    if (p.use_pyr) pyr = *pyr_host;
    dim3 grid(cdiv(max_num, 128), B);
    k_encode_targets<<<grid, 128, 0, (cudaStream_t)stream>>>(p, pyr, tar_box, tar_gt, tar_param, tar_label, tar_is_gt);
    return check_launch("encode_targets");
}

int b2d_roi_targets_fused(int64_t* labels, float* max_iou, long long out_ld, const float* boxes, long long box_ld,
                          const int* box_count, long long N, const float* gt, int gt_ld, const int* gt_count,
                          const int64_t* gt_label, int B, float pos_iou, float neg_iou, float min_pos_iou,
                          int prepend_gt, int* census, int* pos_list, int pos_cap, int* chosen, int* n_chosen,
                          int max_num, int pos_num, unsigned long long seed, const unsigned long long* seed_step,
                          float* tar_box, float* tar_gt, float* tar_param, int64_t* tar_label, int64_t* tar_is_gt,
                          const float* means_host, const float* stds_host, void* stream) {
    B2D_REQUIRE(labels && max_iou && boxes && gt && gt_count && census && chosen && n_chosen, "roi_targets_fused: null pointer");
    B2D_REQUIRE(B >= 1 && gt_ld >= 1 && gt_ld <= kGtChunk && N >= 0 && N <= kSmallThreads * kSmallBoxes,
                "roi_targets_fused: need N <= 4096 and gt_ld <= 512");
    B2D_REQUIRE(max_num >= 1 && max_num <= kSmallThreads && pos_num >= 0 && pos_num <= max_num,
                "roi_targets_fused: need 1 <= max_num <= 1024 and pos_num <= max_num");
    AssignArgs a;
    a.boxes = boxes; a.box_ld = box_ld; a.box_count = box_count; a.N = N;
    a.use_pyr = 0; a.img_hw = nullptr; a.border = 0.0f;
    a.gt = gt; a.gt_ld = gt_ld; a.gt_count = gt_count;
    a.pos_iou = pos_iou; a.neg_iou = neg_iou; a.min_pos_iou = min_pos_iou;
    a.prepend_gt = prepend_gt; a.out_ld = out_ld;
    FusedArgs f;
    f.chosen = chosen; f.n_chosen = n_chosen; f.max_num = max_num; f.pos_num = pos_num; f.seed = seed; f.seed_step = seed_step;
    f.gt_label = gt_label;
    f.tar_box = tar_box; f.tar_gt = tar_gt; f.tar_param = tar_param; f.tar_label = tar_label; f.tar_is_gt = tar_is_gt;
    for (int i = 0; i < 4; ++i) { f.ms[i] = means_host ? means_host[i] : 0.0f; f.ms[4 + i] = stds_host ? stds_host[i] : 1.0f; }
    if (knobs().pdl) {
        cudaLaunchConfig_t cfg;
        memset(&cfg, 0, sizeof(cfg));
        cfg.gridDim = dim3((unsigned)B, 1, 1); cfg.blockDim = dim3(kSmallThreads, 1, 1); cfg.stream = (cudaStream_t)stream;
        cudaLaunchAttribute attr[1];
        attr[0].id = cudaLaunchAttributeProgrammaticStreamSerialization;
        attr[0].val.programmaticStreamSerializationAllowed = 1;
        cfg.attrs = attr; cfg.numAttrs = 1;
        const cudaError_t e = cudaLaunchKernelEx(&cfg, k_roi_targets_small, a, labels, max_iou, census, pos_list, pos_cap, f);
        if (e != cudaSuccess) { set_error(cudaGetErrorString(e)); cudaGetLastError(); return (int)e; }
    } else {
        k_roi_targets_small<<<B, kSmallThreads, 0, (cudaStream_t)stream>>>(a, labels, max_iou, census, pos_list, pos_cap, f);
    }
    return check_launch("roi_targets_fused");
}

}
```

pytorch-faster-rcnn_b200/fused.py:

```python
import ctypes
import os

import numpy as np
import torch

from . import _C


def _ptrs(tensors):
    arr = (_C.c_void_p * _C.MAX_LEVELS)()
    for i, t in enumerate(tensors):
        arr[i] = t.data_ptr()
    return arr


def pinned_channels_last(t):
    B, C, H, W = t.shape
    h = torch.empty((B, H, W, C), dtype=t.dtype, pin_memory=True).permute(0, 3, 1, 2)
    h.copy_(t)
    return h


def _batch_view(obj, b0, b1, rows_per_image=None):
    import copy
    v = copy.copy(obj)
    rows_per_image = rows_per_image or {}
    for k, t in list(vars(obj).items()):
        if isinstance(t, torch.Tensor) and t.dim() >= 1 and k not in ("ws", "step_cell"):
            r = rows_per_image.get(k, 1)
            v.__dict__[k] = t[b0 * r:b1 * r]
    v.B, v.b0 = b1 - b0, getattr(obj, "b0", 0) + b0
    return v


class AnchorPyramid(object):

    def __init__(self, strides, grids, scales=(8,), ratios=(0.5, 1.0, 2.0), center_lt=False):
        self.strides, self.grids = list(strides), [tuple(int(v) for v in g) for g in grids]
        levels = []
        for s, g in zip(self.strides, self.grids):
            ws = [np.float32(s * sc * np.sqrt(ar)) for sc in scales for ar in ratios]
            hs = [np.float32(s * sc / np.sqrt(ar)) for sc in scales for ar in ratios]
            levels.append(dict(stride=s, H=g[0], W=g[1], ws=ws, hs=hs, center_lt=center_lt))
        self.num_anchors = len(scales) * len(ratios)
        self.c = _C.make_pyramid(levels)
        self.total = int(self.c.total)
        self.level_sizes = [self.num_anchors * g[0] * g[1] for g in self.grids]


class RpnProposals(object):

    def __init__(self, pyramid, B, cfg, means, stds, device, score_mode=0, cls_channels=1, do_nms=True,
                 scale_factor=1.0):
        self.pyr, self.B = pyramid, B
        get = (lambda k, d=0: cfg.get(k, d)) if hasattr(cfg, "get") else (lambda k, d=0: getattr(cfg, k, d))
        c = _C.RpnCfg()
        c.pre_nms, c.post_nms, c.max_num = int(get("pre_nms")), int(get("post_nms")), int(get("max_num"))
        c.score_mode, c.num_cls_channels, c.do_nms = int(score_mode), int(cls_channels), int(bool(do_nms))
        c.nms_thr_f = _C.floor_f32(float(get("nms_iou", 0.7)))
        c.min_size = float(np.float32(scale_factor * get("min_bbox_size", 0)))
        for i in range(4):
            c.means[i], c.stds[i] = float(means[i]), float(stds[i])
        self.cfg = c
        nbytes = _C.lib().b2d_rpn_proposals_workspace_bytes(ctypes.byref(self.pyr.c), B, ctypes.byref(c))
        if nbytes == 0:
            raise _C.B200DetError("rpn_proposals: unsupported configuration (a level needs a pre-NMS top-k <= 16384)")
        self.ws = torch.empty(nbytes, dtype=torch.uint8, device=device)
        post = [(c.post_nms if 0 < c.post_nms < k else k) for k in
                [(c.pre_nms if 0 < c.pre_nms < n else n) for n in pyramid.level_sizes]]
        self.P = c.max_num if c.max_num > 0 else sum(post)
        self.props = torch.zeros((B, 4, self.P), dtype=torch.float32, device=device)
        self.scores = torch.zeros((B, self.P), dtype=torch.float32, device=device)
        self.count = torch.zeros(B, dtype=torch.int32, device=device)
        self.prov = torch.zeros((B, self.P), dtype=torch.int32, device=device)
        self.launches = 0

    def slice(self, b0, b1):
        v = _batch_view(self, b0, b1)
        nbytes = _C.lib().b2d_rpn_proposals_workspace_bytes(ctypes.byref(self.pyr.c), v.B, ctypes.byref(self.cfg))
        v.ws = torch.empty(nbytes, dtype=torch.uint8, device=self.ws.device)
        return v

    def __call__(self, cls_outs, reg_outs, img_hw, records=None, targets=None, after_select=None):
        self.cfg.records = records.data_ptr() if records is not None else None
        self.cfg.event_after_select = after_select.cuda_event if after_select is not None else None
        if targets is not None:
            bt, gt, gt_count, gt_label = targets
            ta = bt.target_args(gt, gt_count, gt_label)
            _C.call("b2d_rpn_proposals_targets", _C.ptr(self.props), _C.ptr(self.scores), _C.ptr(self.count), _C.ptr(self.prov),
                    _ptrs(cls_outs), _ptrs(reg_outs), ctypes.byref(self.pyr.c), _C.ptr(img_hw), self.B,
                    ctypes.byref(self.cfg), _C.ptr(self.ws), self.ws.numel(), ctypes.byref(ta), _C.stream())
            self.launches = int(_C.lib().b2d_last_launch_count())
            return self.props, self.scores, self.count
        _C.call("b2d_rpn_proposals", _C.ptr(self.props), _C.ptr(self.scores), _C.ptr(self.count), _C.ptr(self.prov),
                _ptrs(cls_outs), _ptrs(reg_outs), ctypes.byref(self.pyr.c), _C.ptr(img_hw), self.B,
                ctypes.byref(self.cfg), _C.ptr(self.ws), self.ws.numel(), _C.stream())
        self.launches = int(_C.lib().b2d_last_launch_count())
        return self.props, self.scores, self.count


class BatchedTargets(object):

    def __init__(self, B, n_boxes, gt_ld, assigner, sampler, means, stds, device, pyramid=None, border=0.0,
                 prepend_gt=False, seed=0):
        self.B, self.N, self.gt_ld, self.pyr = B, int(n_boxes), int(gt_ld), pyramid
        self.pos_iou, self.neg_iou, self.min_pos = (np.float32(assigner[k]) for k in ("pos_iou", "neg_iou", "min_pos_iou"))
        self.max_num, self.pos_num = int(sampler["max_num"]), int(sampler["pos_num"])
        self.border, self.prepend, self.seed = float(border), int(bool(prepend_gt)), int(seed)
        self.out_ld = self.N + (self.gt_ld if prepend_gt else 0)
        i32, f32, i64 = torch.int32, torch.float32, torch.int64
        self.labels = torch.empty((B, self.out_ld), dtype=i64, device=device)
        self.iou = torch.empty((B, self.out_ld), dtype=f32, device=device)
        self.census = torch.zeros((B, 4), dtype=i32, device=device)
        self.pos_list = torch.empty((B, self.out_ld), dtype=i32, device=device)
        self.colmax = torch.empty((B, self.gt_ld), dtype=i32, device=device)
        self.chosen = torch.empty((B, self.max_num), dtype=i32, device=device)
        self.n_chosen = torch.zeros(B, dtype=i32, device=device)
        self.tar_box = torch.zeros((B, 4, self.max_num), dtype=f32, device=device)
        self.tar_gt = torch.zeros((B, 4, self.max_num), dtype=f32, device=device)
        self.tar_param = torch.zeros((B, 4, self.max_num), dtype=f32, device=device)
        self.tar_label = torch.zeros((B, self.max_num), dtype=i64, device=device)
        self.tar_is_gt = torch.zeros((B, self.max_num), dtype=i64, device=device)
        self.means, self.stds = _C.host_f4(means, [0, 0, 0, 0]), _C.host_f4(stds, [1, 1, 1, 1])
        self.step_cell = torch.zeros(1, dtype=torch.int64, device=device)
        self.auto_bump = True
        self.b0 = 0
        small = pyramid is None and self.N <= 4096 and self.gt_ld <= 512
        self.fused = small and self.max_num <= 1024
        self.launches = 1 if self.fused else (3 if small else (4 if pyramid is not None else 5))

    def reset_step(self):
        self.step_cell.zero_()

    def target_args(self, gt, gt_count, gt_label):
        assert self.fused
        a = _C.RoiTargetArgs()
        dp = lambda t: t.data_ptr() if t is not None else None
        a.labels, a.max_iou, a.out_ld = dp(self.labels), dp(self.iou), self.out_ld
        a.gt, a.gt_ld, a.gt_count, a.gt_label = dp(gt), self.gt_ld, dp(gt_count), dp(gt_label)
        a.pos_iou, a.neg_iou, a.min_pos_iou = float(self.pos_iou), float(self.neg_iou), float(self.min_pos)
        a.prepend_gt, a.census, a.pos_list, a.pos_cap = self.prepend, dp(self.census), dp(self.pos_list), self.out_ld
        a.chosen, a.n_chosen, a.max_num, a.pos_num = dp(self.chosen), dp(self.n_chosen), self.max_num, self.pos_num
        a.seed = (self.seed * 1000003 + 0x632BE59BD9B4E019 * self.b0) & 0xFFFFFFFFFFFFFFFF
        a.seed_step = dp(self.step_cell)
        a.tar_box, a.tar_gt, a.tar_param = dp(self.tar_box), dp(self.tar_gt), dp(self.tar_param)
        a.tar_label, a.tar_is_gt = dp(self.tar_label), dp(self.tar_is_gt)
        for i in range(4):
            a.means[i], a.stds[i] = self.means[i], self.stds[i]
        return a

    def slice(self, b0, b1):
        return _batch_view(self, b0, b1)

    def __call__(self, gt, gt_count, gt_label=None, boxes=None, box_count=None, img_hw=None, tail_stream=None):
        pyr = ctypes.byref(self.pyr.c) if boxes is None else None
        box_ld = boxes.shape[-1] if boxes is not None else 0
        if self.auto_bump:
            _C.call("b2d_counter_add", _C.ptr(self.step_cell), 1, _C.stream())
        base_seed = (self.seed * 1000003 + 0x632BE59BD9B4E019 * self.b0) & 0xFFFFFFFFFFFFFFFF
        if self.fused and boxes is not None:
            _C.call("b2d_roi_targets_fused", _C.ptr(self.labels), _C.ptr(self.iou), self.out_ld, _C.ptr(boxes), box_ld,
                    _C.ptr(box_count), self.N, _C.ptr(gt), self.gt_ld, _C.ptr(gt_count), _C.ptr(gt_label), self.B,
                    float(self.pos_iou), float(self.neg_iou), float(self.min_pos), self.prepend, _C.ptr(self.census),
                    _C.ptr(self.pos_list), self.out_ld, _C.ptr(self.chosen), _C.ptr(self.n_chosen), self.max_num,
                    self.pos_num, base_seed, _C.ptr(self.step_cell),
                    _C.ptr(self.tar_box), _C.ptr(self.tar_gt), _C.ptr(self.tar_param), _C.ptr(self.tar_label),
                    _C.ptr(self.tar_is_gt), self.means, self.stds, _C.stream())
            return self
        _C.call("b2d_assign_max_iou", _C.ptr(self.labels), _C.ptr(self.iou), self.out_ld, _C.ptr(boxes), box_ld,
                _C.ptr(box_count), self.N, pyr, _C.ptr(img_hw), self.border, _C.ptr(gt), self.gt_ld, _C.ptr(gt_count),
                self.B, float(self.pos_iou), float(self.neg_iou), float(self.min_pos), self.prepend,
                _C.ptr(self.census), _C.ptr(self.pos_list), self.out_ld, _C.ptr(self.colmax), self.colmax.numel() * 4,
                _C.stream())
        cnt, cnt_add = (box_count, gt_count) if (self.prepend and box_count is not None) else \
            ((None, gt_count) if self.prepend else (box_count, None))
        n = self.N if cnt is None else 0
        if tail_stream is not None:
            tail_stream.wait_stream(torch.cuda.current_stream())
            with torch.cuda.stream(tail_stream):
                self._sample_encode(cnt, cnt_add, n, base_seed, boxes, box_ld, pyr, gt, gt_count, gt_label)
            return self
        self._sample_encode(cnt, cnt_add, n, base_seed, boxes, box_ld, pyr, gt, gt_count, gt_label)
        return self

    def _sample_encode(self, cnt, cnt_add, n, base_seed, boxes, box_ld, pyr, gt, gt_count, gt_label):
        _C.call("b2d_sample_labels", _C.ptr(self.chosen), _C.ptr(self.n_chosen), _C.ptr(self.labels), self.out_ld,
                _C.ptr(cnt), _C.ptr(cnt_add), n, _C.ptr(self.census), _C.ptr(self.pos_list), self.out_ld, self.B,
                self.max_num, self.pos_num, base_seed, _C.ptr(self.step_cell), _C.stream())
        _C.call("b2d_encode_targets", _C.ptr(self.tar_box), _C.ptr(self.tar_gt), _C.ptr(self.tar_param),
                _C.ptr(self.tar_label), _C.ptr(self.tar_is_gt), _C.ptr(self.chosen), _C.ptr(self.n_chosen),
                self.max_num, _C.ptr(self.labels), self.out_ld, _C.ptr(boxes), box_ld, pyr, _C.ptr(gt), self.gt_ld,
                _C.ptr(gt_count), _C.ptr(gt_label), self.prepend, self.means, self.stds, self.B, _C.stream())
        return self


class BatchedRoIAlign(object):

    def __init__(self, B, ld, feat_shapes, strides, device, out_size=(7, 7), sampling_ratio=2, finest_scale=56,
                 layout=1):
        cfg = _C.RoiCfg()
        cfg.num_levels, cfg.C = len(strides), int(feat_shapes[0][0])
        cfg.PH, cfg.PW, cfg.sampling_ratio, cfg.aligned = int(out_size[0]), int(out_size[1]), int(sampling_ratio), 0
        cfg.layout, cfg.finest_scale = int(layout), float(finest_scale)
        for l, (s, shp) in enumerate(zip(strides, feat_shapes)):
            cfg.H[l], cfg.W[l], cfg.spatial_scale[l] = int(shp[1]), int(shp[2]), 1.0 / float(s)
        self.cfg, self.B, self.ld = cfg, B, ld
        self.out = torch.zeros((B * ld, cfg.C, cfg.PH, cfg.PW), dtype=torch.float32, device=device)
        self.launches = 1

    def slice(self, b0, b1):
        return _batch_view(self, b0, b1, rows_per_image={"out": self.ld})

    def __call__(self, feats, rois, counts):
        _C.call("b2d_roi_align_fwd_batched", _C.ptr(self.out), _ptrs(feats), _C.ptr(rois), self.ld, _C.ptr(counts),
                self.B, ctypes.byref(self.cfg), _C.stream())
        return self.out

    def fetch_touched(self, dev_feats, host_feats, rois, counts):
        if not hasattr(self, "_bitmap"):
            n = _C.lib().b2d_roi_cell_bitmap_bytes(self.B, ctypes.byref(self.cfg))
            self._bitmap = torch.zeros(n, dtype=torch.uint8, device=self.out.device)
            self.cells_moved = torch.zeros(1, dtype=torch.int64, device=self.out.device)
        for d, h in zip(dev_feats, host_feats):
            if not (h.is_pinned() and d.is_cuda and d.shape == h.shape and d.dtype == h.dtype and d.stride() == h.stride()
                    and h.is_contiguous(memory_format=torch.channels_last)):
                raise _C.B200DetError("fetch_touched: host maps must be pinned channels_last tensors matching the device maps")
        _C.call("b2d_roi_mark_cells", _C.ptr(self._bitmap), _C.ptr(rois), self.ld, _C.ptr(counts), self.B,
                ctypes.byref(self.cfg), _C.stream())
        _C.call("b2d_fetch_marked_cells", _ptrs(dev_feats), _ptrs(host_feats), _C.ptr(self._bitmap), self.B,
                ctypes.byref(self.cfg), _C.ptr(self.cells_moved), _C.stream())
        return self.cells_moved


class TrainHotPath(object):

    def __init__(self, B, grids, device, strides=(4, 8, 16, 32, 64), gt_ld=64, feat_channels=256,
                 rpn_proposal=None, rpn_assigner=None, rpn_sampler=None, rcnn_assigner=None, rcnn_sampler=None,
                 rpn_stds=(1.0, 1.0, 1.0, 1.0), rcnn_stds=(0.1, 0.1, 0.2, 0.2), allowed_border=0, layout=1, seed=0,
                 groups=1, overlap=False, order=None):
        z4 = (0.0, 0.0, 0.0, 0.0)
        self.order = order or os.environ.get("B2D_STEP_ORDER", "rpn_first")
        self.ev_select = torch.cuda.Event()
        self.ev_select.record()
        self.fuse_targets = os.environ.get("B2D_FUSE_TARGETS", "0") != "0"
        rpn_proposal = rpn_proposal or dict(pre_nms=2000, post_nms=2000, max_num=2000, nms_iou=0.7, min_bbox_size=0)
        rpn_assigner = rpn_assigner or dict(pos_iou=0.7, neg_iou=0.3, min_pos_iou=0.3)
        rpn_sampler = rpn_sampler or dict(max_num=256, pos_num=128)
        rcnn_assigner = rcnn_assigner or dict(pos_iou=0.5, neg_iou=0.5, min_pos_iou=0.5)
        rcnn_sampler = rcnn_sampler or dict(max_num=512, pos_num=128)
        self.B, self.device = B, device
        self.pyr = AnchorPyramid(strides, grids)
        self.proposals = RpnProposals(self.pyr, B, rpn_proposal, z4, rpn_stds, device)
        self.rpn_targets = BatchedTargets(B, self.pyr.total, gt_ld, rpn_assigner, rpn_sampler, z4, rpn_stds, device,
                                          pyramid=self.pyr, border=allowed_border, seed=seed)
        self.roi_targets = BatchedTargets(B, self.proposals.P, gt_ld, rcnn_assigner, rcnn_sampler, z4, rcnn_stds,
                                          device, prepend_gt=True, seed=seed + 1)
        self.step_cell = torch.ones(1, dtype=torch.int64, device=device)
        self.s_bump = torch.cuda.Stream(device=device)
        for t in (self.rpn_targets, self.roi_targets):
            t.step_cell, t.auto_bump = self.step_cell, False
        roi_strides = list(strides[:4])
        shapes = [(feat_channels, g[0], g[1]) for g in grids[:4]]
        self.roi_align = BatchedRoIAlign(B, rcnn_sampler["max_num"], shapes, roi_strides, device, layout=layout)
        m = rpn_sampler["max_num"]
        self.tar_cls = torch.zeros((B, 1, m), dtype=torch.float32, device=device)
        self.tar_reg = torch.zeros((B, 4, m), dtype=torch.float32, device=device)
        groups = max(1, min(int(groups), B))
        while B % groups:
            groups -= 1
        self.groups = groups
        self.subs = []
        if groups > 1 or overlap:
            per = B // groups
            for g in range(groups):
                b0, b1 = g * per, (g + 1) * per
                self.subs.append((b0, b1, self.proposals.slice(b0, b1) if groups > 1 else self.proposals,
                                  self.roi_targets.slice(b0, b1) if groups > 1 else self.roi_targets,
                                  self.roi_align.slice(b0, b1) if groups > 1 else self.roi_align,
                                  torch.cuda.Stream(device=device, priority=-4 + min(g, 2)),
                                  torch.cuda.Stream(device=device, priority=-2 + min(g, 1))))
            self.s_rpn = torch.cuda.Stream(device=device, priority=int(os.environ.get("B2D_RPN_PRIO", "0")))
            tp = os.environ.get("B2D_RPN_TAIL_PRIO", "")
            self.s_tail = torch.cuda.Stream(device=device, priority=int(tp)) if tp else None
        self.launches = 0

    def reset_step(self):
        self.step_cell.fill_(1)

    def _rpn_target_chain(self, cls_outs, reg_outs, gt, gt_count, img_hw):
        tail = getattr(self, "s_tail", None)
        rt = self.rpn_targets(gt, gt_count, None, img_hw=img_hw, tail_stream=tail)
        cur = torch.cuda.current_stream()
        with torch.cuda.stream(tail if tail is not None else cur):
            _C.call("b2d_gather_head_outputs", _C.ptr(self.tar_cls), _C.ptr(self.tar_reg), _ptrs(cls_outs), _ptrs(reg_outs),
                    ctypes.byref(self.pyr.c), 1, _C.ptr(rt.chosen), _C.ptr(rt.n_chosen), rt.max_num, self.B, _C.stream())
        if tail is not None:
            cur.wait_stream(tail)
        return rt

    def step(self, cls_outs, reg_outs, feats, gt, gt_count, gt_label, img_hw, feats_ready=None, records=None,
             before_roi_align=None):
        if not self.subs:
            if feats_ready is not None:
                torch.cuda.current_stream().wait_event(feats_ready)
            ride = self.roi_targets.fused and self.fuse_targets
            props, scores, count = self.proposals(cls_outs, reg_outs, img_hw, records=records,
                                                  targets=(self.roi_targets, gt, gt_count, gt_label) if ride else None)
            rt = self._rpn_target_chain(cls_outs, reg_outs, gt, gt_count, img_hw)
            bt = self.roi_targets if ride else self.roi_targets(gt, gt_count, gt_label, boxes=props, box_count=count)
            _C.call("b2d_counter_add", _C.ptr(self.step_cell), 1, _C.stream())
            if before_roi_align is not None:
                before_roi_align(bt.tar_box, bt.n_chosen)
            self.roi_align(feats, bt.tar_box, bt.n_chosen)
        else:
            cur = torch.cuda.current_stream()
            rpn_first = self.order == "rpn_first"
            self.s_rpn.wait_stream(cur)
            if rpn_first:
                with torch.cuda.stream(self.s_rpn):
                    rt = self._rpn_target_chain(cls_outs, reg_outs, gt, gt_count, img_hw)
            for gi, (b0, b1, prop, tgt, ra, st, st_lo) in enumerate(self.subs):
                st.wait_stream(cur)
                ride = tgt.fused and self.fuse_targets
                ev = self.ev_select if (gi == 0 and self.order == "rpn_after_select") else None
                with torch.cuda.stream(st):
                    p, _, c = prop([t[b0:b1] for t in cls_outs], [t[b0:b1] for t in reg_outs], img_hw[b0:b1],
                                   records=records[b0:b1] if records is not None else None,
                                   targets=(tgt, gt[b0:b1], gt_count[b0:b1], gt_label[b0:b1]) if ride else None,
                                   after_select=ev)
                if gi == 0 and not rpn_first:
                    if self.order == "rpn_late":
                        self.s_rpn.wait_stream(st)
                    if ev is not None:
                        self.s_rpn.wait_event(ev)
                    with torch.cuda.stream(self.s_rpn):
                        rt = self._rpn_target_chain(cls_outs, reg_outs, gt, gt_count, img_hw)
                with torch.cuda.stream(st):
                    t2 = tgt if ride else tgt(gt[b0:b1], gt_count[b0:b1], gt_label[b0:b1], boxes=p, box_count=c)
                st_lo.wait_stream(st)
                if feats_ready is not None:
                    st_lo.wait_event(feats_ready)
                with torch.cuda.stream(st_lo):
                    if before_roi_align is not None:
                        if self.groups != 1:
                            raise _C.B200DetError("before_roi_align needs groups == 1")
                        before_roi_align(t2.tar_box, t2.n_chosen)
                    ra([f[b0:b1] for f in feats], t2.tar_box, t2.n_chosen)
            for sub in self.subs:
                self.s_bump.wait_stream(sub[-2])
            self.s_bump.wait_stream(self.s_rpn)
            with torch.cuda.stream(self.s_bump):
                _C.call("b2d_counter_add", _C.ptr(self.step_cell), 1, _C.stream())
            for sub in self.subs:
                cur.wait_stream(sub[-1])
            cur.wait_stream(self.s_rpn)
            cur.wait_stream(self.s_bump)
        self.launches = (sum(sub[2].launches for sub in self.subs) if self.groups > 1 else self.proposals.launches) + \
            ((0 if (self.roi_targets.fused and self.fuse_targets) else self.roi_targets.launches) + 1) * self.groups + \
            self.rpn_targets.launches + 1 + 1
        return dict(props=self.proposals.props, scores=self.proposals.scores, prop_count=self.proposals.count,
                    rpn=self.rpn_targets, rpn_tar_cls=self.tar_cls, rpn_tar_reg=self.tar_reg, rcnn=self.roi_targets,
                    roi_feats=self.roi_align.out)

    def step_from_host(self, h_cls, h_reg, h_feats, h_gt, h_gt_label, gt_count, img_hw, h_out=None,
                       with_roi_feats=False, sparse=None):
        dev, B = self.device, self.B
        cl = all(t.dim() == 4 and t.is_contiguous(memory_format=torch.channels_last) and not t.is_contiguous()
                 for t in h_feats)
        if sparse is None:
            sparse = cl and all(t.is_pinned() for t in h_feats)
        if sparse:
            return self._step_from_host_sparse(h_cls, h_reg, h_feats, h_gt, h_gt_label, gt_count, img_hw, h_out,
                                               with_roi_feats)
        if not hasattr(self, "_stage"):
            st = dict(cls=[torch.empty(t.shape, dtype=t.dtype, device=dev) for t in h_cls],
                      reg=[torch.empty(t.shape, dtype=t.dtype, device=dev) for t in h_reg],
                      feat=[torch.empty(t.shape, dtype=t.dtype, device=dev) for t in h_feats],
                      nhwc=[torch.empty(t.shape, dtype=t.dtype, device=dev).contiguous(memory_format=torch.channels_last)
                            for t in h_feats],
                      gt=torch.empty(h_gt.shape, dtype=h_gt.dtype, device=dev),
                      gl=torch.empty(h_gt_label.shape, dtype=h_gt_label.dtype, device=dev),
                      s_copy=torch.cuda.Stream(device=dev), s_xpose=torch.cuda.Stream(device=dev, priority=0),
                      ev_heads=torch.cuda.Event(), ev_feat=[torch.cuda.Event() for _ in h_feats],
                      ev_ready=torch.cuda.Event())
            self._stage = st
        st = self._stage
        if h_out is None:
            h_out = self._host_results(with_roi_feats)
        cur = torch.cuda.current_stream()
        sc, sx = st["s_copy"], st["s_xpose"]
        sc.wait_stream(cur)
        sx.wait_stream(cur)
        with torch.cuda.stream(sc):
            st["gt"].copy_(h_gt, non_blocking=True)
            st["gl"].copy_(h_gt_label, non_blocking=True)
            for d, h in zip(st["cls"] + st["reg"], list(h_cls) + list(h_reg)):
                d.copy_(h, non_blocking=True)
            st["ev_heads"].record(sc)
            for l in sorted(range(len(h_feats)), key=lambda i: -h_feats[i].numel()):
                st["feat"][l].copy_(h_feats[l], non_blocking=True)
                st["ev_feat"][l].record(sc)
        with torch.cuda.stream(sx):
            for l in sorted(range(len(h_feats)), key=lambda i: -h_feats[i].numel()):
                sx.wait_event(st["ev_feat"][l])
                f = st["feat"][l]
                _C.call("b2d_nchw_to_nhwc", _C.ptr(st["nhwc"][l]), _C.ptr(f), f.shape[0], f.shape[1], f.shape[2],
                        f.shape[3], _C.stream())
            st["ev_ready"].record(sx)
        cur.wait_event(st["ev_heads"])
        out = self.step(st["cls"], st["reg"], st["nhwc"], st["gt"], gt_count, st["gl"], img_hw, feats_ready=st["ev_ready"])
        return self._read_back(out, h_out)

    def _host_results(self, with_roi_feats):
        if not hasattr(self, "_h_out"):
            pin = lambda t: torch.empty(t.shape, dtype=t.dtype).pin_memory()
            rt, bt = self.rpn_targets, self.roi_targets
            self._h_out = dict(props=pin(self.proposals.props), scores=pin(self.proposals.scores),
                               prop_count=pin(self.proposals.count), rpn_label=pin(rt.tar_label),
                               rpn_param=pin(rt.tar_param), rpn_tar_cls=pin(self.tar_cls), rpn_tar_reg=pin(self.tar_reg),
                               roi_label=pin(bt.tar_label), roi_param=pin(bt.tar_param), roi_count=pin(bt.n_chosen),
                               roi_probe=torch.empty(1).pin_memory())
        if with_roi_feats and "roi_feats" not in self._h_out:
            self._h_out["roi_feats"] = torch.empty(self.roi_align.out.shape, dtype=self.roi_align.out.dtype).pin_memory()
        return self._h_out

    @staticmethod
    def _read_back(out, h_out):
        pairs = [("props", out["props"]), ("scores", out["scores"]), ("prop_count", out["prop_count"]),
                 ("rpn_label", out["rpn"].tar_label), ("rpn_param", out["rpn"].tar_param),
                 ("rpn_tar_cls", out["rpn_tar_cls"]), ("rpn_tar_reg", out["rpn_tar_reg"]),
                 ("roi_label", out["rcnn"].tar_label), ("roi_param", out["rcnn"].tar_param),
                 ("roi_count", out["rcnn"].n_chosen), ("roi_feats", out["roi_feats"]),
                 ("roi_probe", out["roi_feats"][0, 0, 0, :1])]
        for k, t in pairs:
            if k in h_out:
                h_out[k].copy_(t, non_blocking=True)
        return h_out

    def _step_from_host_sparse(self, h_cls, h_reg, h_feats, h_gt, h_gt_label, gt_count, img_hw, h_out, with_roi_feats):
        dev = self.device
        if self.groups != 1:
            raise _C.B200DetError("step_from_host(sparse): image groups are not supported")
        if not hasattr(self, "_stage_sparse"):
            self._stage_sparse = dict(
                cls=[torch.empty(t.shape, dtype=t.dtype, device=dev) for t in h_cls],
                reg=None,
                nhwc=[torch.zeros(t.shape, dtype=t.dtype, device=dev).contiguous(memory_format=torch.channels_last)
                      for t in h_feats],
                gt=torch.empty(h_gt.shape, dtype=h_gt.dtype, device=dev),
                gl=torch.empty(h_gt_label.shape, dtype=h_gt_label.dtype, device=dev),
                s_copy=torch.cuda.Stream(device=dev), ev_heads=torch.cuda.Event())
        st = self._stage_sparse
        if h_out is None:
            h_out = self._host_results(with_roi_feats)
        cur = torch.cuda.current_stream()
        sc = st["s_copy"]
        sc.wait_stream(cur)
        zc_reg = getattr(self, "reg_zero_copy", True) and all(t.is_pinned() and t.is_contiguous() for t in h_reg)
        if not zc_reg and st["reg"] is None:
            st["reg"] = [torch.empty(t.shape, dtype=t.dtype, device=dev) for t in h_reg]
        with torch.cuda.stream(sc):
            st["gt"].copy_(h_gt, non_blocking=True)
            st["gl"].copy_(h_gt_label, non_blocking=True)
            for d, h in zip(st["cls"] + ([] if zc_reg else st["reg"]), list(h_cls) + ([] if zc_reg else list(h_reg))):
                d.copy_(h, non_blocking=True)
            st["ev_heads"].record(sc)
        cur.wait_event(st["ev_heads"])
        fetch = lambda rois, counts: self.roi_align.fetch_touched(st["nhwc"], h_feats, rois, counts)
        out = self.step(st["cls"], list(h_reg) if zc_reg else st["reg"], st["nhwc"], st["gt"], gt_count, st["gl"], img_hw,
                        before_roi_align=fetch)
        self.last_reg_zero_copy = zc_reg
        return self._read_back(out, h_out)


class CascadeHotPath(object):

    def __init__(self, B, n_props, grids, device, strides=(4, 8, 16, 32), gt_ld=64, feat_channels=256,
                 thresholds=(0.5, 0.6, 0.7),
                 stage_stds=((0.1, 0.1, 0.2, 0.2), (0.05, 0.05, 0.1, 0.1), (0.033, 0.033, 0.067, 0.067)),
                 sampler=None, num_classes=21, layout=1, seed=0):
        sampler = sampler or dict(max_num=512, pos_num=128)
        z4 = (0.0, 0.0, 0.0, 0.0)
        self.B, self.m, self.C = B, int(sampler["max_num"]), int(num_classes)
        shapes = [(feat_channels, g[0], g[1]) for g in grids[:len(strides)]]
        self.stages = []
        n = int(n_props)
        for s, (thr, sd) in enumerate(zip(thresholds, stage_stds)):
            tg = BatchedTargets(B, n, gt_ld, dict(pos_iou=thr, neg_iou=thr, min_pos_iou=thr), sampler, z4, sd, device,
                                prepend_gt=True, seed=seed + s)
            ra = BatchedRoIAlign(B, self.m, shapes, list(strides), device, layout=layout)
            refined = torch.zeros((B, 4, self.m), dtype=torch.float32, device=device)
            rcount = torch.zeros(B, dtype=torch.int32, device=device)
            self.stages.append((tg, ra, refined, rcount, _C.host_f4(sd, [1, 1, 1, 1])))
            n = self.m
        self.step_cell = torch.zeros(1, dtype=torch.int64, device=device)
        for st in self.stages:
            st[0].step_cell, st[0].auto_bump = self.step_cell, False
        self.roi_img = torch.arange(B, dtype=torch.int32, device=device).repeat_interleave(self.m).contiguous()
        self.rois_flat = [torch.zeros((4, B * self.m), dtype=torch.float32, device=device) for _ in self.stages]
        mf = torch.channels_last if layout != 0 else torch.contiguous_format
        self.grads = [[torch.zeros((B,) + shp, dtype=torch.float32, device=device).contiguous(memory_format=mf) for shp in shapes]
                      for _ in self.stages]
        self.bwd_cfg = self.stages[0][1].cfg
        nb = _C.lib().b2d_roi_align_bwd_workspace_bytes(B * self.m, B, ctypes.byref(self.bwd_cfg))
        self.bwd_ws = torch.empty(nb, dtype=torch.uint8, device=device)
        self.zero4 = _C.host_f4(z4, [0, 0, 0, 0])
        self.launches = len(self.stages) * (1 + 1 + 1) + 1

    def step(self, props, prop_count, feats, gt, gt_count, gt_label, img_hw, reg_outs):
        outs = []
        boxes, count = props, prop_count
        _C.call("b2d_counter_add", _C.ptr(self.step_cell), 1, _C.stream())
        for s, (tg, ra, refined, rcount, stds) in enumerate(self.stages):
            bt = tg(gt, gt_count, gt_label, boxes=boxes, box_count=count)
            ra(feats, bt.tar_box, bt.n_chosen)
            _C.call("b2d_refine_bboxes", _C.ptr(refined), _C.ptr(rcount), _C.ptr(bt.tar_box), self.m, _C.ptr(bt.n_chosen),
                    self.m, _C.ptr(bt.tar_label), _C.ptr(reg_outs[s]), self.C, _C.ptr(bt.tar_is_gt), self.zero4, stds, 1,
                    _C.ptr(img_hw), self.B, _C.stream())
            outs.append((bt, ra.out, refined, rcount))
            boxes, count = refined, rcount
        return outs

    def backward(self, grad_feats):
        for s, (tg, ra, _, _, _) in enumerate(self.stages):
            self.rois_flat[s].copy_(tg.tar_box.permute(1, 0, 2).reshape(4, -1))
            arr = (_C.c_void_p * _C.MAX_LEVELS)()
            for i, g in enumerate(self.grads[s]):
                arr[i] = g.data_ptr()
            _C.call("b2d_roi_align_bwd", arr, _C.ptr(grad_feats[s]), _C.ptr(self.rois_flat[s]), self.B * self.m,
                    _C.ptr(self.roi_img), None, self.B * self.m, self.B, ctypes.byref(self.bwd_cfg), _C.ptr(self.bwd_ws),
                    self.bwd_ws.numel(), _C.stream())
        return self.grads


class InferHotPath(object):

    def __init__(self, B, grids, device, strides=(4, 8, 16, 32, 64), feat_channels=256, num_classes=21, num_stages=1,
                 rpn_test=None, rcnn_test=None,
                 stage_stds=((0.1, 0.1, 0.2, 0.2), (0.05, 0.05, 0.1, 0.1), (0.033, 0.033, 0.067, 0.067)),
                 reg_class_agnostic=False, layout=1):
        rpn_test = rpn_test or dict(pre_nms=1000, post_nms=1000, max_num=1000, nms_iou=0.7, min_bbox_size=0)
        rcnn_test = rcnn_test or dict(min_score=0.05, nms_iou=0.5, max_per_img=100, nms_type='official')
        if not 1 <= num_stages <= len(stage_stds):
            raise ValueError("num_stages must be in 1..%d (one stds tuple per stage)" % len(stage_stds))
        z4 = (0.0, 0.0, 0.0, 0.0)
        self.B, self.device, self.S = B, device, int(num_stages)
        self.NC, self.reg_c = int(num_classes), 1 if reg_class_agnostic else int(num_classes)
        self.pyr = AnchorPyramid(strides, grids)
        self.proposals = RpnProposals(self.pyr, B, rpn_test, z4, (1.0, 1.0, 1.0, 1.0), device)
        self.P = P = self.proposals.P
        shapes = [(feat_channels, g[0], g[1]) for g in grids[:4]]
        self.roi_align = [BatchedRoIAlign(B, P, shapes, list(strides[:4]), device, layout=layout) for _ in range(self.S)]
        self.stds = [_C.host_f4(sd, [1, 1, 1, 1]) for sd in stage_stds[:self.S]]
        self.zero4 = _C.host_f4(z4, [0, 0, 0, 0])
        self.boxes = [torch.zeros((B, 4, P), dtype=torch.float32, device=device) for _ in range(self.S - 1)]
        self.counts = [torch.zeros(B, dtype=torch.int32, device=device) for _ in range(self.S - 1)]
        get = (lambda k, d=None: rcnn_test.get(k, d)) if hasattr(rcnn_test, "get") else (lambda k, d=None: getattr(rcnn_test, k, d))
        mode = get('nms_type', 'official')
        self.min_score, self.nms_thr = float(np.float32(get('min_score'))), _C.floor_f32(float(get('nms_iou')))
        self.strict = int(mode == 'strict')
        self.cap = max(1, min(16384, P * ((self.NC - 1) if not self.strict else 1)))
        mpi = get('max_per_img')
        self.M = M = max(1, min(int(mpi) if mpi is not None else self.cap, self.cap))
        self.det_box = torch.zeros((B, 4, M), dtype=torch.float32, device=device)
        self.det_score = torch.zeros((B, M), dtype=torch.float32, device=device)
        self.det_label = torch.zeros((B, M), dtype=torch.int64, device=device)
        self.det_count = torch.zeros(B, dtype=torch.int32, device=device)
        self.overflow = torch.zeros(1, dtype=torch.int32, device=device)
        self.det_ws = torch.empty(_C.lib().b2d_rcnn_detect_workspace_bytes(self.cap, B), dtype=torch.uint8, device=device)

    def step(self, cls_outs, reg_outs, feats, img_hw, heads, records=None, mark=None):
        if records is not None and (tuple(records.shape) != (self.B, self.M, 6) or records.dtype != torch.float32
                                    or not records.is_contiguous()):
            raise _C.B200DetError("InferHotPath.step: records must be contiguous fp32 [%d, %d, 6]" % (self.B, self.M))
        props, _, count = self.proposals(cls_outs, reg_outs, img_hw)
        if mark is not None:
            mark("proposals")
        boxes, stages = props, []
        for s in range(self.S):
            roi_feats = self.roi_align[s](feats, boxes, count)
            if mark is not None:
                mark("roi_align%d" % s)
            cls_out, reg_out = heads[s](roi_feats)
            cls_out, reg_out = _C.f32c(cls_out), _C.f32c(reg_out)
            if tuple(cls_out.shape) != (self.B * self.P, self.NC) or tuple(reg_out.shape) != (self.B * self.P, 4 * self.reg_c):
                raise _C.B200DetError("InferHotPath.step: stage %d head returned %s / %s, expected [%d, %d] / [%d, %d]"
                                      % (s, tuple(cls_out.shape), tuple(reg_out.shape), self.B * self.P, self.NC,
                                         self.B * self.P, 4 * self.reg_c))
            if mark is not None:
                mark("head%d" % s)
            stages.append(dict(boxes=boxes, count=count, roi_feats=roi_feats, cls_out=cls_out, reg_out=reg_out))
            if s + 1 < self.S:
                _C.call("b2d_refine_bboxes_argmax", _C.ptr(self.boxes[s]), _C.ptr(self.counts[s]), _C.ptr(boxes), self.P,
                        _C.ptr(count), self.P, _C.ptr(cls_out), self.NC, _C.ptr(reg_out), self.reg_c, self.zero4,
                        self.stds[s], _C.ptr(img_hw), self.B, _C.stream())
                boxes, count = self.boxes[s], self.counts[s]
                if mark is not None:
                    mark("refine%d" % s)
        last = stages[-1]
        args = [_C.ptr(self.det_box), _C.ptr(self.det_score), _C.ptr(self.det_label), _C.ptr(self.det_count)]
        if records is not None:
            args.append(_C.ptr(records))
        args += [_C.ptr(boxes), self.P, _C.ptr(count), self.P, _C.ptr(last["cls_out"]), _C.ptr(last["reg_out"]), self.NC,
                 self.reg_c, self.zero4, self.stds[-1], _C.ptr(img_hw), self.min_score, self.nms_thr, self.M, self.strict,
                 self.cap, self.B, _C.ptr(self.overflow), _C.ptr(self.det_ws), self.det_ws.numel(), _C.stream()]
        _C.call("b2d_rcnn_detect_records" if records is not None else "b2d_rcnn_detect", *args)
        if mark is not None:
            mark("detect")
        return dict(boxes=self.det_box, scores=self.det_score, labels=self.det_label, count=self.det_count,
                    records=records, stages=stages)

    def check(self):
        torch.cuda.synchronize(self.device)
        if int(self.overflow[0]):
            raise _C.B200DetError("rcnn_detect: more than 16384 (box, class) candidates; raise min_score")


class DenseInferHotPath(object):

    def __init__(self, B, grids, device, head="retina", num_classes=21, test_cfg=None, strides=(8, 16, 32, 64, 128),
                 use_sigmoid=True, anchor_scales=tuple(4 * 2 ** (i / 3) for i in range(3)), anchor_ratios=(0.5, 1.0, 2.0),
                 center_lt=False, target_means=(0.0, 0.0, 0.0, 0.0), target_stds=(1.0, 1.0, 1.0, 1.0), reg_mean=0.0,
                 reg_std=300.0, use_centerness=True, scale_factor=1.0):
        if head not in ("retina", "fcos"):
            raise _C.B200DetError("DenseInferHotPath: head must be 'retina' or 'fcos', got %r" % (head,))
        test_cfg = test_cfg or dict(pre_nms=1000, min_bbox_size=0, min_score=0.05, nms_iou=0.5, max_per_img=100,
                                    nms_type="strict")
        get = (lambda k, d=None: test_cfg.get(k, d)) if hasattr(test_cfg, "get") else (lambda k, d=None: getattr(test_cfg, k, d))
        mode = get("nms_type", "official")
        if mode not in ("official", "strict"):
            raise _C.B200DetError("DenseInferHotPath: nms_type must be 'official' or 'strict'")
        self.B, self.device, self.head = int(B), device, head
        self.grids = [tuple(int(v) for v in g) for g in grids]
        self.L = len(self.grids)
        sigmoid = head == "fcos" or bool(use_sigmoid)
        self.C = C = int(num_classes) - 1 if sigmoid else int(num_classes)
        if not 1 <= C <= 128:
            raise _C.B200DetError("DenseInferHotPath: 1..128 class channels supported, got %d" % C)
        self.pre = int(get("pre_nms", 0) or 0)
        min_bbox = float(get("min_bbox_size", 0) or 0)
        self.min_score = float(np.float32(get("min_score", -1)))
        self.nms_thr = _C.floor_f32(float(get("nms_iou")))
        self.strict = int(mode == "strict")
        chans = list(range(0, C)) if sigmoid else list(range(1, C))
        mask = [0, 0]
        for c in chans:
            mask[c >> 6] |= 1 << (c & 63)
        self.chan = (_C.c_ull * 2)(*mask)
        self.label_add = 1 if sigmoid else 0
        self.lv = _C.DenseLevels()
        if head == "retina":
            self.transform = 1 if sigmoid else 2
            self.pyr = AnchorPyramid(strides, self.grids, tuple(anchor_scales), tuple(anchor_ratios), center_lt)
            self.A = self.pyr.num_anchors
            sel_cfg = dict(pre_nms=self.pre, post_nms=0, max_num=0, nms_iou=0.5, min_bbox_size=min_bbox)
            self.select = RpnProposals(self.pyr, B, sel_cfg, target_means, target_stds, device,
                                       score_mode=2 if sigmoid else 3, cls_channels=C, do_nms=False, scale_factor=scale_factor)
            self.P = self.select.P
            self.lv.num_levels = self.L
            for l, n in enumerate(self.pyr.level_sizes):
                self.lv.offset[l], self.lv.img_stride[l], self.lv.class_stride[l] = int(self.pyr.c.lv[l].offset), C * n, n
        else:
            from . import heads
            self.transform, self.centerness = 0, bool(use_centerness)
            self.pyr_c = heads._point_pyramid(self.grids, strides, 8)
            self.total = T = int(self.pyr_c.total)
            sizes = [h * w for h, w in self.grids]
            self.sizes = (_C.c_int * _C.MAX_LEVELS)(*sizes)
            self.P = sum(min(self.pre, n) if self.pre > 0 else n for n in sizes)
            self.reg_mean, self.reg_std = float(reg_mean), float(reg_std)
            self.min_size = float(np.float32(scale_factor * min_bbox))
            self.boxes = torch.zeros((B, 4, T), dtype=torch.float32, device=device)
            self.key = torch.zeros((B, T), dtype=torch.float32, device=device)
            self.score = torch.zeros((B, C, T), dtype=torch.float32, device=device)
            self.ctrs = torch.zeros((B, T), dtype=torch.float32, device=device) if self.centerness else None
            self.sel_idx = torch.zeros((B, self.P), dtype=torch.int32, device=device)
            self.sel_count = torch.zeros(B, dtype=torch.int32, device=device)
            self.sel_boxes = torch.zeros((B, 4, self.P), dtype=torch.float32, device=device)
            nb = _C.lib().b2d_dense_select_workspace_bytes(self.sizes, self.L, B, self.pre)
            if nb == 0:
                raise _C.B200DetError("DenseInferHotPath: unsupported selection (1..8 levels, a level top-k <= 16384)")
            self.sel_ws = torch.empty(nb, dtype=torch.uint8, device=device)
            self.lv.num_levels = 1
            self.lv.offset[0], self.lv.img_stride[0], self.lv.class_stride[0] = 0, C * T, T
            self.lv.base[0] = self.score.data_ptr()
        self.cap = max(1, min(16384, self.P * (len(chans) if not self.strict else 1)))
        mpi = get("max_per_img")
        self.M = M = max(1, min(int(mpi) if mpi is not None else self.cap, self.cap))
        self.det_box = torch.zeros((B, 4, M), dtype=torch.float32, device=device)
        self.det_score = torch.zeros((B, M), dtype=torch.float32, device=device)
        self.det_label = torch.zeros((B, M), dtype=torch.int64, device=device)
        self.det_count = torch.zeros(B, dtype=torch.int32, device=device)
        self.overflow = torch.zeros(1, dtype=torch.int32, device=device)
        self.det_ws = torch.empty(_C.lib().b2d_rcnn_detect_workspace_bytes(self.cap, B), dtype=torch.uint8, device=device)

    def _check_maps(self, what, maps, per_cell):
        if maps is None or len(maps) != self.L:
            raise _C.B200DetError("DenseInferHotPath.step: %s needs %d levels" % (what, self.L))
        for (h, w), t in zip(self.grids, maps):
            if (tuple(t.shape) != (self.B, per_cell, h, w) or t.dtype != torch.float32 or not t.is_contiguous()
                    or not t.is_cuda):
                raise _C.B200DetError("DenseInferHotPath.step: %s level of shape %s (%s), expected contiguous fp32 CUDA "
                                      "[%d, %d, %d, %d]" % (what, tuple(t.shape), t.dtype, self.B, per_cell, h, w))

    def step(self, cls_outs, reg_outs, img_hw, ctr_outs=None, records=None, mark=None, detect_events=None):
        B = self.B
        if tuple(img_hw.shape) != (B, 2) or img_hw.dtype != torch.float32 or not img_hw.is_contiguous():
            raise _C.B200DetError("DenseInferHotPath.step: img_hw must be contiguous fp32 [%d, 2]" % B)
        if records is not None and (tuple(records.shape) != (B, self.M, 6) or records.dtype != torch.float32
                                    or not records.is_contiguous()):
            raise _C.B200DetError("DenseInferHotPath.step: records must be contiguous fp32 [%d, %d, 6]" % (B, self.M))
        if self.head == "retina":
            self._check_maps("cls_outs", cls_outs, self.A * self.C)
            self._check_maps("reg_outs", reg_outs, 4 * self.A)
            boxes, count, rows = self.select(cls_outs, reg_outs, img_hw)[0], self.select.count, self.select.prov
            for l, t in enumerate(cls_outs):
                self.lv.base[l] = t.data_ptr()
            factor = None
            if mark is not None:
                mark("selection")
        else:
            self._check_maps("cls_outs", cls_outs, self.C)
            self._check_maps("reg_outs", reg_outs, 4)
            if self.centerness:
                self._check_maps("ctr_outs", ctr_outs, 1)
            _C.call("b2d_fcos_decode", _C.ptr(self.boxes), _C.ptr(self.key), _C.ptr(self.score), _C.ptr(self.ctrs),
                    _ptrs(cls_outs), _ptrs(reg_outs), _ptrs(ctr_outs) if self.centerness else None, ctypes.byref(self.pyr_c),
                    self.C, self.reg_mean, self.reg_std, self.min_size, _C.ptr(img_hw), B, _C.stream())
            if mark is not None:
                mark("decode")
            _C.call("b2d_dense_select", _C.ptr(self.sel_idx), _C.ptr(self.sel_count), _C.ptr(self.sel_boxes), _C.ptr(self.key),
                    _C.ptr(self.boxes), self.sizes, self.L, B, self.pre, _C.ptr(self.sel_ws), self.sel_ws.numel(), _C.stream())
            boxes, count, rows, factor = self.sel_boxes, self.sel_count, self.sel_idx, self.ctrs
            if mark is not None:
                mark("selection")
        ev = None
        if detect_events is not None:
            ev = (_C.c_void_p * 2)(*[e.cuda_event for e in detect_events])
        args = [_C.ptr(self.det_box), _C.ptr(self.det_score), _C.ptr(self.det_label), _C.ptr(self.det_count)]
        if records is not None:
            args.append(_C.ptr(records))
        args += [_C.ptr(boxes), self.P, _C.ptr(count), _C.ptr(rows), ctypes.byref(self.lv), self.C, self.transform,
                 _C.ptr(factor), self.total if factor is not None else 0, self.chan, self.min_score, self.label_add,
                 self.nms_thr, self.M, self.strict, self.cap, B, _C.ptr(self.overflow), _C.ptr(self.det_ws),
                 self.det_ws.numel(), ev, _C.stream()]
        _C.call("b2d_dense_detect_records" if records is not None else "b2d_dense_detect", *args)
        if mark is not None:
            mark("detect")
        return dict(boxes=self.det_box, scores=self.det_score, labels=self.det_label, count=self.det_count,
                    records=records, sel_boxes=boxes, sel_count=count, sel_rows=rows)

    def check(self):
        torch.cuda.synchronize(self.device)
        if int(self.overflow[0]):
            raise _C.B200DetError("dense_detect: more than 16384 (box, class) candidates in an image; raise min_score")
```

Before: 32730.

## Add sparse RPN anchor assignment that labels only anchors near ground-truth boxes

```diff
diff --git a/include/b200det.h b/include/b200det.h
--- a/include/b200det.h
+++ b/include/b200det.h
@@ -53,6 +53,15 @@
                        const float* img_hw, float border, const float* gt, int gt_ld, const int* gt_count,
                        int B, float pos_iou, float neg_iou, float min_pos_iou, int prepend_gt, int* census,
                        int* pos_list, int pos_cap, void* workspace, size_t ws_bytes, void* stream);
+
+B2D_API int b2d_assign_sparse(int* census, int* pos_list, int pos_cap, const b2d_pyramid* pyr_host, const float* img_hw,
+                      float border, const float* gt, int gt_ld, const int* gt_count, int B, float pos_iou,
+                      float neg_iou, float min_pos_iou, void* workspace, size_t ws_bytes, void* stream);
+B2D_API int b2d_sample_labels_sparse(int* chosen, int* n_chosen, int64_t* labels, long long ld, const int* census,
+                      const int* pos_list, int pos_cap, const b2d_pyramid* pyr_host, const float* img_hw, float border,
+                      const float* gt, int gt_ld, const int* gt_count, const void* workspace, int B, float pos_iou,
+                      float neg_iou, float min_pos_iou, int max_num, int pos_num, unsigned long long seed,
+                      const unsigned long long* seed_step, void* stream);
 
 B2D_API int b2d_sample_labels(int* chosen, int* n_chosen, const int64_t* labels, long long ld, const int* count,
                       const int* count_add , long long n, const int* census, const int* pos_list, int pos_cap, int B, int max_num,
diff --git a/pytorch-faster-rcnn_b200/_C.py b/pytorch-faster-rcnn_b200/_C.py
--- a/pytorch-faster-rcnn_b200/_C.py
+++ b/pytorch-faster-rcnn_b200/_C.py
@@ -67,6 +67,10 @@
                            c_float, c_float, c_int, _P, _P, c_int, _P, c_size_t, _P],
     "b2d_sample_labels": [_P, _P, _P, c_ll, _P, _P, c_ll, _P, _P, c_int, c_int, c_int, c_int, c_ull, _P, _P],
     "b2d_counter_add": [_P, c_ull, _P],
+    "b2d_assign_sparse": [_P, _P, c_int, _P, _P, c_float, _P, c_int, _P, c_int, c_float, c_float, c_float, _P, c_size_t,
+                          _P],
+    "b2d_sample_labels_sparse": [_P, _P, _P, c_ll, _P, _P, c_int, _P, _P, c_float, _P, c_int, _P, _P, c_int, c_float,
+                                 c_float, c_float, c_int, c_int, c_ull, _P, _P],
     "b2d_roi_targets_fused": [_P, _P, c_ll, _P, c_ll, _P, c_ll, _P, c_int, _P, _P, c_int, c_float, c_float, c_float,
                               c_int, _P, _P, c_int, _P, _P, c_int, c_int, c_ull, _P, _P, _P, _P, _P, _P, _P, _P, _P],
     "b2d_anchor_loss_fwd": [_P, _P, _P, _P, _P, c_ll, _P, c_int, _P, c_int, c_float, c_float, c_float, _P, _P, c_int, _P,
diff --git a/pytorch-faster-rcnn_b200/csrc/assign.cu b/pytorch-faster-rcnn_b200/csrc/assign.cu
--- a/pytorch-faster-rcnn_b200/csrc/assign.cu
+++ b/pytorch-faster-rcnn_b200/csrc/assign.cu
@@ -198,12 +198,100 @@
 
 constexpr int kRowAnchors = 4;
 
+struct LabelGt {
+    Box t; float ta, cm;
+    bool all;
+};
+
+__device__ __forceinline__ LabelGt label_gt(const Box& t, uint32_t colmax_key, int j, float min_pos_iou) {
+    LabelGt g;
+    g.t = t; g.ta = area_plus1(t);
+    g.cm = colmax_key ? fmaxf(key2f(colmax_key), 0.0f) : 0.0f;
+    g.all = j == 0 || (g.cm >= min_pos_iou && g.cm == 0.0f) || !(g.ta > 0.0f);
+    return g;
+}
+
+struct LabelAcc {
+    float best, veq; int arg, eq;
+};
+
+__device__ __forceinline__ void label_init(LabelAcc& s) { s.best = 0.0f; s.veq = 0.0f; s.arg = 0; s.eq = -1; }
+
+__device__ __forceinline__ void label_step(LabelAcc& s, const Box& bx, float ba, const LabelGt& g, int j,
+                                           float min_pos_iou) {
+    const bool hit = fmaxf(bx.x1, g.t.x1) < fminf(bx.x2, g.t.x2) && fmaxf(bx.y1, g.t.y1) < fminf(bx.y2, g.t.y2);
+    if (!(hit || g.all || !(ba > 0.0f))) return;
+    const float v = iou_plus1(bx, ba, g.t, g.ta);
+    if (j == 0 || v > s.best) { s.best = v; s.arg = j; }
+    if (s.eq < 0 && g.cm >= min_pos_iou && v == g.cm) { s.eq = j; s.veq = v; }
+}
+
+__device__ __forceinline__ int label_final(const LabelAcc& s, float pos_iou, float neg_iou, float* iou, int* gt) {
+    int lb = -1;
+    if (s.best < neg_iou) lb = 0;
+    if (s.best >= pos_iou) lb = 1;
+    int a = s.arg;
+    *iou = s.best;
+    if (s.eq >= 0) { lb = 1; a = s.eq; *iou = s.veq; }
+    *gt = a;
+    return (lb == 1) ? a + 1 : lb;
+}
+
+__device__ __forceinline__ void gt_cell_rect(const b2d_level& lv, int a, const Box& t, float ta,
+                                             int& x0, int& x1, int& y0, int& y1) {
+    const float s = lv.stride;
+    const float hw = lv.ws[a] / 2.0f, hh = lv.hs[a] / 2.0f, off = lv.center_lt ? 0.0f : s / 2.0f;
+    x0 = 0; x1 = lv.W - 1; y0 = 0; y1 = lv.H - 1;
+    if (ta > 0.0f) {
+        x0 = max(0, (int)floorf((t.x1 - hw - off) / s) - 1);
+        x1 = min(lv.W - 1, (int)ceilf((t.x2 + hw - off) / s) + 1);
+        y0 = max(0, (int)floorf((t.y1 - hh - off) / s) - 1);
+        y1 = min(lv.H - 1, (int)ceilf((t.y2 + hh - off) / s) + 1);
+    }
+}
+
+__device__ __forceinline__ bool axis_valid(float lo, float hi, int c, int in_c, float img_c, float border) {
+    return c < in_c && (!(border >= 0.0f) || (lo >= -border && hi < img_c + border));
+}
+
 __device__ __forceinline__ bool anchor_valid(const AssignArgs& p, const Box& a, int y, int x, int in_h, int in_w,
                                              float img_h, float img_w) {
-    bool ok = (y < in_h) && (x < in_w);
-    if (p.border >= 0.0f)
-        ok = ok && a.x1 >= -p.border && a.y1 >= -p.border && a.x2 < img_w + p.border && a.y2 < img_h + p.border;
-    return ok;
+    return axis_valid(a.x1, a.x2, x, in_w, img_w, p.border) && axis_valid(a.y1, a.y2, y, in_h, img_h, p.border);
+}
+
+constexpr int kSparseMaxGt = 4096;
+
+__device__ __forceinline__ void stage_label_gts(const AssignArgs& p, const uint32_t* __restrict__ colmax, int b,
+                                                LabelGt* s_g) {
+    const float* g = p.gt + (long long)b * 4 * p.gt_ld;
+    for (int j = threadIdx.x; j < p.gt_count[b]; j += blockDim.x) {
+        const Box t{g[j], g[p.gt_ld + j], g[2 * p.gt_ld + j], g[3 * p.gt_ld + j]};
+        s_g[j] = label_gt(t, colmax[(long long)b * p.gt_ld + j], j, p.min_pos_iou);
+    }
+}
+
+__device__ __forceinline__ int anchor_label(const AssignArgs& p, const LabelGt* s_g, int K, const Box& bx, float ba,
+                                            float* iou, int* gt) {
+    LabelAcc acc;
+    label_init(acc);
+    for (int j = 0; j < K; ++j) label_step(acc, bx, ba, s_g[j], j, p.min_pos_iou);
+    return label_final(acc, p.pos_iou, p.neg_iou, iou, gt);
+}
+
+__device__ __forceinline__ int anchor_label_at(const AssignArgs& p, const b2d_pyramid& pyr, const int* s_lim,
+                                               const LabelGt* s_g, int K, int b, long long i) {
+    int l = 0;
+    for (int q = 1; q < pyr.num_levels; ++q) if (i >= pyr.lv[q].offset) l = q;
+    const b2d_level& lv = pyr.lv[l];
+    const int li = (int)(i - lv.offset), hw = lv.H * lv.W;
+    const int a = li / hw, r = li - a * hw;
+    const int y = r / lv.W, x = r - y * lv.W;
+    const float img_h = p.img_hw[2 * b], img_w = p.img_hw[2 * b + 1];
+    const Box bx = anchor_at(lv, a, y, x);
+    if (!anchor_valid(p, bx, y, x, s_lim[2 * l], s_lim[2 * l + 1], img_h, img_w)) return -1;
+    float v;
+    int gj;
+    return anchor_label(p, s_g, K, bx, area_plus1(bx), &v, &gj);
 }
 
 constexpr int kRectChunks = 4;
@@ -226,15 +314,8 @@
     const float img_h = p.img_hw[2 * b], img_w = p.img_hw[2 * b + 1];
     int in_h, in_w;
     grid_limits(lv, img_h, img_w, in_h, in_w);
-    const float s = lv.stride;
-    const float hw = lv.ws[a] / 2.0f, hh = lv.hs[a] / 2.0f, off = lv.center_lt ? 0.0f : s / 2.0f;
-    int x0 = 0, x1 = lv.W - 1, y0 = 0, y1 = lv.H - 1;
-    if (ta > 0.0f) {
-        x0 = max(0, (int)floorf((t.x1 - hw - off) / s) - 1);
-        x1 = min(lv.W - 1, (int)ceilf((t.x2 + hw - off) / s) + 1);
-        y0 = max(0, (int)floorf((t.y1 - hh - off) / s) - 1);
-        y1 = min(lv.H - 1, (int)ceilf((t.y2 + hh - off) / s) + 1);
-    }
+    int x0, x1, y0, y1;
+    gt_cell_rect(lv, a, t, ta, x0, x1, y0, y1);
     const int rw = x1 - x0 + 1;
     uint32_t m = 0u;
     if (rw > 0) {
@@ -259,10 +340,7 @@
 __global__ void __launch_bounds__(256) k_label_rows(AssignArgs p, b2d_pyramid pyr, const uint32_t* __restrict__ colmax,
                                                     int64_t* __restrict__ labels, float* __restrict__ out_iou,
                                                     int* __restrict__ census, int* __restrict__ pos_list, int pos_cap) {
-    __shared__ Box s_gt[kGtChunk];
-    __shared__ float s_ga[kGtChunk];
-    __shared__ float s_cm[kGtChunk];
-    __shared__ unsigned char s_all[kGtChunk];
+    __shared__ LabelGt s_g[kGtChunk];
     __shared__ int s_cnt[2];
     const int b = blockIdx.y;
     const int K = p.gt_count[b];
@@ -271,8 +349,8 @@
     if (threadIdx.x < 2) s_cnt[threadIdx.x] = 0;
     const long long i0 = ((long long)blockIdx.x * blockDim.x + threadIdx.x) * kRowAnchors;
     Box bx[kRowAnchors];
-    float ba[kRowAnchors], best[kRowAnchors], veq[kRowAnchors];
-    int arg[kRowAnchors], eq[kRowAnchors];
+    float ba[kRowAnchors];
+    LabelAcc acc[kRowAnchors];
     bool ok[kRowAnchors], live[kRowAnchors];
     float ylo = INFINITY, yhi = -INFINITY;
     {
@@ -303,36 +381,23 @@
             }
             ba[q] = ok[q] ? area_plus1(bx[q]) : 0.0f;
             if (ok[q]) { ylo = fminf(ylo, bx[q].y1); yhi = fmaxf(yhi, bx[q].y2); }
-            best[q] = 0.0f; veq[q] = 0.0f; arg[q] = 0; eq[q] = -1;
+            label_init(acc[q]);
         }
     }
     for (int j0 = 0; j0 < K; j0 += kGtChunk) {
         const int kc = min(kGtChunk, K - j0);
         __syncthreads();
         for (int j = threadIdx.x; j < kc; j += blockDim.x) {
-            Box t{g[j0 + j], g[p.gt_ld + j0 + j], g[2 * p.gt_ld + j0 + j], g[3 * p.gt_ld + j0 + j]};
-            const float ta = area_plus1(t);
-            const uint32_t ck = colmax[(long long)b * p.gt_ld + j0 + j];
-            const float cm = ck ? fmaxf(key2f(ck), 0.0f) : 0.0f;
-            s_gt[j] = t; s_ga[j] = ta; s_cm[j] = cm;
-            s_all[j] = ((j0 + j) == 0 || (cm >= p.min_pos_iou && cm == 0.0f) || !(ta > 0.0f)) ? 1 : 0;
+            const Box t{g[j0 + j], g[p.gt_ld + j0 + j], g[2 * p.gt_ld + j0 + j], g[3 * p.gt_ld + j0 + j]};
+            s_g[j] = label_gt(t, colmax[(long long)b * p.gt_ld + j0 + j], j0 + j, p.min_pos_iou);
         }
         __syncthreads();
         for (int j = 0; j < kc; ++j) {
-            const Box t = s_gt[j];
-            const bool all = s_all[j] != 0;
-            if (!all && !(fmaxf(ylo, t.y1) < fminf(yhi, t.y2))) continue;
-            const float ta = s_ga[j], cm = s_cm[j];
-            const bool cm_ok = cm >= p.min_pos_iou;
-#pragma unroll
-            for (int q = 0; q < kRowAnchors; ++q) {
-                if (!ok[q]) continue;
-                const bool hit = fmaxf(bx[q].x1, t.x1) < fminf(bx[q].x2, t.x2) && fmaxf(bx[q].y1, t.y1) < fminf(bx[q].y2, t.y2);
-                if (!(hit || all || !(ba[q] > 0.0f))) continue;
-                const float v = iou_plus1(bx[q], ba[q], t, ta);
-                if ((j0 + j) == 0 || v > best[q]) { best[q] = v; arg[q] = j0 + j; }
-                if (eq[q] < 0 && cm_ok && v == cm) { eq[q] = j0 + j; veq[q] = v; }
-            }
+            const LabelGt gj = s_g[j];
+            if (!gj.all && !(fmaxf(ylo, gj.t.y1) < fminf(yhi, gj.t.y2))) continue;
+#pragma unroll
+            for (int q = 0; q < kRowAnchors; ++q)
+                if (ok[q]) label_step(acc[q], bx[q], ba[q], gj, j0 + j, p.min_pos_iou);
         }
     }
     int64_t* lab = labels + (long long)b * p.out_ld;
@@ -343,15 +408,8 @@
 #pragma unroll
     for (int q = 0; q < kRowAnchors; ++q) {
         ol[q] = -1; ov[q] = 0.0f;
-        if (ok[q]) {
-            int lb = -1;
-            if (best[q] < p.neg_iou) lb = 0;
-            if (best[q] >= p.pos_iou) lb = 1;
-            int a = arg[q];
-            ov[q] = best[q];
-            if (eq[q] >= 0) { lb = 1; a = eq[q]; ov[q] = veq[q]; }
-            ol[q] = (lb == 1) ? (int64_t)(a + 1) : (int64_t)lb;
-        }
+        int a;
+        if (ok[q]) ol[q] = label_final(acc[q], p.pos_iou, p.neg_iou, &ov[q], &a);
     }
     const bool vec = live[kRowAnchors - 1] && ((reinterpret_cast<uintptr_t>(lab) & 15) == 0) &&
                      ((reinterpret_cast<uintptr_t>(oiou) & 15) == 0);
@@ -379,6 +437,89 @@
     }
     __syncthreads();
     if (threadIdx.x < 2 && s_cnt[threadIdx.x]) atomicAdd(&census[4 * b + threadIdx.x], s_cnt[threadIdx.x]);
+}
+
+__global__ void __launch_bounds__(256, 4) k_label_rect(AssignArgs p, b2d_pyramid pyr, const uint32_t* __restrict__ colmax,
+                                                    int max_a, int n_rect, int* __restrict__ census,
+                                                    int* __restrict__ pos_list, int pos_cap) {
+    extern __shared__ LabelGt s_g[];
+    __shared__ int s_red[2][8];
+    const int b = blockIdx.y;
+    const float img_h = p.img_hw[2 * b], img_w = p.img_hw[2 * b + 1];
+    int c0 = 0, c1 = 0;
+    const bool count_blk = (int)blockIdx.x >= n_rect;
+    if (count_blk) {
+        const int w = blockIdx.x - n_rect;
+        const int a = w % max_a, l = w / max_a;
+        const b2d_level& lv = pyr.lv[l];
+        if (a >= lv.A) return;
+        int in_h, in_w;
+        grid_limits(lv, img_h, img_w, in_h, in_w);
+        for (int x = threadIdx.x; x < lv.W; x += blockDim.x) {
+            const Box an = anchor_at(lv, a, 0, x);
+            c0 += axis_valid(an.x1, an.x2, x, in_w, img_w, p.border);
+        }
+        for (int y = threadIdx.x; y < lv.H; y += blockDim.x) {
+            const Box an = anchor_at(lv, a, y, 0);
+            c1 += axis_valid(an.y1, an.y2, y, in_h, img_h, p.border);
+        }
+    } else {
+        int w = blockIdx.x;
+        const int rc = w % kRectChunks; w /= kRectChunks;
+        const int a = w % max_a; w /= max_a;
+        const int l = w % pyr.num_levels;
+        const int j = w / pyr.num_levels;
+        const int K = p.gt_count[b];
+        if (j >= K) return;
+        const b2d_level& lv = pyr.lv[l];
+        if (a >= lv.A) return;
+        stage_label_gts(p, colmax, b, s_g);
+        __syncthreads();
+        const Box t = s_g[j].t;
+        const bool degen = !(s_g[j].ta > 0.0f);
+        const float min_iou = fminf(fminf(p.pos_iou, p.neg_iou), p.min_pos_iou);
+        int in_h, in_w;
+        grid_limits(lv, img_h, img_w, in_h, in_w);
+        int x0, x1, y0, y1;
+        gt_cell_rect(lv, a, t, s_g[j].ta, x0, x1, y0, y1);
+        int* plist = pos_list + (long long)b * pos_cap;
+        const int tx = threadIdx.x % 64, ty = threadIdx.x / 64;
+        for (int y = y0 + rc + ty * kRectChunks; y <= y1; y += 4 * kRectChunks) {
+            for (int xb = x0; xb <= x1; xb += 64) {
+                const int x = xb + tx;
+                bool pos = false;
+                if (x <= x1) {
+                    const Box an = anchor_at(lv, a, y, x);
+                    const float aa = area_plus1(an);
+                    const bool cand = degen || !(iou_plus1(an, aa, t, s_g[j].ta) < min_iou);
+                    if (cand && anchor_valid(p, an, y, x, in_h, in_w, img_h, img_w)) {
+                        float v;
+                        int gj;
+                        const int lb = anchor_label(p, s_g, K, an, aa, &v, &gj);
+                        if (lb != 0 && gj == j) { ++c1; pos = lb > 0; }
+                    }
+                }
+                const int slot = warp_alloc(pos, &census[4 * b + 2]);
+                if (pos) {
+                    ++c0;
+                    if (slot < pos_cap) plist[slot] = (int)(lv.offset + ((long long)a * lv.H + y) * lv.W + x);
+                }
+            }
+        }
+    }
+    c0 = __reduce_add_sync(0xffffffffu, c0);
+    c1 = __reduce_add_sync(0xffffffffu, c1);
+    if (lane_id() == 0) { s_red[0][threadIdx.x >> 5] = c0; s_red[1][threadIdx.x >> 5] = c1; }
+    __syncthreads();
+    if (threadIdx.x == 0) {
+        for (int q = 1; q < 8; ++q) { c0 += s_red[0][q]; c1 += s_red[1][q]; }
+        if (count_blk) {
+            if (c0 * c1) atomicAdd(&census[4 * b + 1], c0 * c1);
+        } else {
+            if (c0) atomicAdd(&census[4 * b + 0], c0);
+            if (c1) atomicSub(&census[4 * b + 1], c1);
+        }
+    }
 }
 
 __device__ __forceinline__ void assign_small_body(const AssignArgs& p, SmallSmem& sm, int64_t* __restrict__ labels,
@@ -521,20 +662,40 @@
 constexpr int kSampleThreads = 1024;
 constexpr int kSampleSortCap = 4096;
 
-__global__ void __launch_bounds__(kSampleThreads) k_sample(int* __restrict__ chosen, int* __restrict__ n_chosen,
+struct SparseSample {
+    AssignArgs p; const uint32_t* colmax; int64_t* labels;
+};
+constexpr size_t kSampleSortBytes = (size_t)kSampleSortCap * 8;
+
+template <bool kSparse>
+__global__ void __launch_bounds__(kSparse ? kSampleThreads / 2 : kSampleThreads) k_sample(int* __restrict__ chosen, int* __restrict__ n_chosen,
                                                            const int64_t* __restrict__ labels, long long ld,
                                                            const int* __restrict__ count,
                                                            const int* __restrict__ count_add, long long n,
                                                            const int* __restrict__ census,
                                                            const int* __restrict__ pos_list, int pos_cap,
                                                            int max_num, int pos_num, unsigned long long seed,
-                                                           const unsigned long long* __restrict__ seed_step) {
+                                                           const unsigned long long* __restrict__ seed_step,
+                                                           SparseSample sp, b2d_pyramid pyr) {
     extern __shared__ __align__(16) uint64_t s_sort[];
     if (seed_step) seed += *seed_step;
     __shared__ int s_n, s_warp[kSampleThreads / 32], s_take;
     __shared__ unsigned long long s_lo, s_hi;
     const int b = blockIdx.x;
     const int64_t* lab = labels + (long long)b * ld;
+    LabelGt* s_g = reinterpret_cast<LabelGt*>(reinterpret_cast<unsigned char*>(s_sort) + kSampleSortBytes);
+    const int K = kSparse ? sp.p.gt_count[b] : 0;
+    __shared__ int s_lim[2 * kMaxLevels];
+    if constexpr (kSparse) {
+        stage_label_gts(sp.p, sp.colmax, b, s_g);
+        if (threadIdx.x < pyr.num_levels)
+            grid_limits(pyr.lv[threadIdx.x], sp.p.img_hw[2 * b], sp.p.img_hw[2 * b + 1], s_lim[2 * threadIdx.x],
+                        s_lim[2 * threadIdx.x + 1]);
+    }
+    auto is_neg = [&](uint32_t y) -> bool {
+        if constexpr (kSparse) return anchor_label_at(sp.p, pyr, s_lim, s_g, K, b, (long long)y) == 0;
+        return lab[y] == 0;
+    };
     const long long n_b = (count ? (long long)count[b] : n) + (count_add ? (long long)count_add[b] : 0);
     const int npos = min(census[4 * b + 0], pos_cap);
     const int nneg = census[4 * b + 1];
@@ -603,7 +764,7 @@
                 for (int q = 0; q < 4; ++q) {
                     const long long t = t0 + (long long)q * blockDim.x + threadIdx.x;
                     y[q] = feistel((uint32_t)t, half, sd ^ 0xA5A5A5A5DEADBEEFull);
-                    hit[q] = t < dom && ((long long)y[q] < n_b) && (lab[y[q]] == 0);
+                    hit[q] = t < dom && ((long long)y[q] < n_b) && is_neg(y[q]);
                 }
 #pragma unroll
                 for (int q = 0; q < 4; ++q) {
@@ -627,7 +788,7 @@
         } else
         for (long long t0 = 0; t0 < dom; t0 += blockDim.x) {
             const uint32_t y = feistel((uint32_t)(t0 + threadIdx.x), half, sd ^ 0xA5A5A5A5DEADBEEFull);
-            const bool hit = ((long long)y < n_b) && (lab[y] == 0);
+            const bool hit = ((long long)y < n_b) && is_neg(y);
             const unsigned m = __ballot_sync(0xffffffffu, hit);
             if (lane_id() == 0) s_warp[threadIdx.x >> 5] = __popc(m);
             __syncthreads();
@@ -653,8 +814,11 @@
         s_sort[t] = (t < total) ? (0xffffffffull - s_sort[t]) + 1ull : 0ull;
     __syncthreads();
     bitonic_sort_desc(s_sort, p2);
-    for (int t = threadIdx.x; t < max_num; t += blockDim.x)
-        out[t] = (t < total) ? (int)(0xffffffffull - (s_sort[t] - 1ull)) : -1;
+    for (int t = threadIdx.x; t < max_num; t += blockDim.x) {
+        const int idx = (t < total) ? (int)(0xffffffffull - (s_sort[t] - 1ull)) : -1;
+        out[t] = idx;
+        if constexpr (kSparse) if (t < total) sp.labels[(long long)b * ld + idx] = anchor_label_at(sp.p, pyr, s_lim, s_g, K, b, idx);
+    }
     if (threadIdx.x == 0) n_chosen[b] = total;
 }
 
@@ -772,6 +936,40 @@
     if (i < n) p[i] = v;
 }
 
+static bool sparse_ok(const b2d_pyramid* pyr, float pos_iou, float neg_iou, float min_pos_iou) {
+    if (!(pos_iou > 0.0f && neg_iou > 0.0f && min_pos_iou > 0.0f)) return false;
+    for (int l = 0; l < pyr->num_levels; ++l)
+        for (int a = 0; a < pyr->lv[l].A; ++a)
+            if (!(pyr->lv[l].ws[a] > 0.0f && pyr->lv[l].hs[a] > 0.0f)) return false;
+    return true;
+}
+
+static AssignArgs sparse_args(const float* img_hw, float border, const float* gt, int gt_ld, const int* gt_count,
+                              float pos_iou, float neg_iou, float min_pos_iou, long long total) {
+    AssignArgs a;
+    memset(&a, 0, sizeof(a));
+    a.N = total; a.use_pyr = 1; a.img_hw = img_hw; a.border = border;
+    a.gt = gt; a.gt_ld = gt_ld; a.gt_count = gt_count;
+    a.pos_iou = pos_iou; a.neg_iou = neg_iou; a.min_pos_iou = min_pos_iou;
+    a.out_ld = total;
+    return a;
+}
+
+template <bool kSparse>
+static int launch_sample(int* chosen, int* n_chosen, const int64_t* labels, long long ld, const int* count,
+                         const int* count_add, long long n, const int* census, const int* pos_list, int pos_cap, int B,
+                         int max_num, int pos_num, unsigned long long seed, const unsigned long long* seed_step,
+                         const SparseSample& sp, const b2d_pyramid& pyr, void* stream) {
+    const size_t smem = kSampleSortBytes + (kSparse ? sizeof(LabelGt) * sp.p.gt_ld : 0);
+    B2D_SMEM(k_sample<kSparse>, smem, "k_sample");
+    const int threads = (knobs().sample_threads == 128 || knobs().sample_threads == 256) ? knobs().sample_threads
+                      : (kSparse ? kSampleThreads / 2 : kSampleThreads);
+    k_sample<kSparse><<<B, threads, smem, (cudaStream_t)stream>>>(
+        chosen, n_chosen, labels, ld, count, count_add, n, census, pos_list, pos_cap, max_num, pos_num, seed, seed_step,
+        sp, pyr);
+    return check_launch("sample_labels");
+}
+
 }
 
 using namespace b2d;
@@ -842,11 +1040,59 @@
     B2D_REQUIRE(B >= 1 && max_num >= 1 && max_num <= kSampleSortCap && pos_num >= 0 && pos_num <= max_num,
                 "sample_labels: need 1 <= max_num <= 4096 and pos_num <= max_num");
     B2D_REQUIRE(n < (1ll << 31), "sample_labels: n too large");
-    B2D_SMEM(k_sample, kSampleSortCap * 8, "k_sample");
-    const int threads = (knobs().sample_threads == 128 || knobs().sample_threads == 256) ? knobs().sample_threads : kSampleThreads;
-    k_sample<<<B, threads, kSampleSortCap * 8, (cudaStream_t)stream>>>(
-        chosen, n_chosen, labels, ld, count, count_add, n, census, pos_list, pos_cap, max_num, pos_num, seed, seed_step);
-    return check_launch("sample_labels");
+    SparseSample sp;
+    memset(&sp, 0, sizeof(sp));
+    b2d_pyramid pyr;
+    memset(&pyr, 0, sizeof(pyr));
+    return launch_sample<false>(chosen, n_chosen, labels, ld, count, count_add, n, census, pos_list, pos_cap, B, max_num,
+                                pos_num, seed, seed_step, sp, pyr, stream);
+}
+
+int b2d_assign_sparse(int* census, int* pos_list, int pos_cap, const b2d_pyramid* pyr_host, const float* img_hw,
+                      float border, const float* gt, int gt_ld, const int* gt_count, int B, float pos_iou, float neg_iou,
+                      float min_pos_iou, void* workspace, size_t ws_bytes, void* stream) {
+    B2D_REQUIRE(census && pos_list && pyr_host && img_hw && gt && gt_count, "assign_sparse: null pointer");
+    B2D_REQUIRE(B >= 1 && gt_ld >= 1 && gt_ld <= kSparseMaxGt && pos_cap >= pyr_host->total,
+                "assign_sparse: need 1 <= gt_ld <= 4096 and pos_cap >= the anchors per image");
+    B2D_REQUIRE(workspace && ws_bytes >= (size_t)B * gt_ld * 4, "assign_sparse: workspace too small");
+    B2D_REQUIRE(sparse_ok(pyr_host, pos_iou, neg_iou, min_pos_iou), "assign_sparse: need pos_iou, neg_iou, min_pos_iou > 0 "
+                "and anchor shapes of positive width and height");
+    cudaStream_t st = (cudaStream_t)stream;
+    const b2d_pyramid& pyr = *pyr_host;
+    AssignArgs a = sparse_args(img_hw, border, gt, gt_ld, gt_count, pos_iou, neg_iou, min_pos_iou, pyr.total);
+    uint32_t* cmx = (uint32_t*)workspace;
+    cudaMemsetAsync(census, 0, sizeof(int) * 4 * B, st);
+    cudaMemsetAsync(cmx, 0, sizeof(uint32_t) * (size_t)B * gt_ld, st);
+    int max_a = 1;
+    for (int l = 0; l < pyr.num_levels; ++l) max_a = max(max_a, pyr.lv[l].A);
+    const int n_rect = gt_ld * pyr.num_levels * max_a * kRectChunks;
+    k_colmax_rect<<<dim3(n_rect, B), 256, 0, st>>>(a, pyr, cmx, max_a);
+    const size_t smem = sizeof(LabelGt) * gt_ld;
+    B2D_SMEM(k_label_rect, smem, "k_label_rect");
+    k_label_rect<<<dim3(n_rect + pyr.num_levels * max_a, B), 256, smem, st>>>(a, pyr, cmx, max_a, n_rect, census, pos_list,
+                                                                              pos_cap);
+    return check_launch("assign_sparse");
+}
+
+int b2d_sample_labels_sparse(int* chosen, int* n_chosen, int64_t* labels, long long ld, const int* census,
+                             const int* pos_list, int pos_cap, const b2d_pyramid* pyr_host, const float* img_hw,
+                             float border, const float* gt, int gt_ld, const int* gt_count, const void* workspace, int B,
+                             float pos_iou, float neg_iou, float min_pos_iou, int max_num, int pos_num,
+                             unsigned long long seed, const unsigned long long* seed_step, void* stream) {
+    B2D_REQUIRE(chosen && n_chosen && labels && census && pos_list && pyr_host && img_hw && gt && gt_count && workspace,
+                "sample_labels_sparse: null pointer");
+    B2D_REQUIRE(B >= 1 && max_num >= 1 && max_num <= kSampleSortCap && pos_num >= 0 && pos_num <= max_num,
+                "sample_labels_sparse: need 1 <= max_num <= 4096 and pos_num <= max_num");
+    B2D_REQUIRE(pyr_host->total < (1ll << 31) && ld >= pyr_host->total && gt_ld >= 1 && gt_ld <= kSparseMaxGt,
+                "sample_labels_sparse: need ld >= the anchors per image and 1 <= gt_ld <= 4096");
+    B2D_REQUIRE(sparse_ok(pyr_host, pos_iou, neg_iou, min_pos_iou), "sample_labels_sparse: need pos_iou, neg_iou, "
+                "min_pos_iou > 0 and anchor shapes of positive width and height");
+    SparseSample sp;
+    sp.p = sparse_args(img_hw, border, gt, gt_ld, gt_count, pos_iou, neg_iou, min_pos_iou, pyr_host->total);
+    sp.colmax = (const uint32_t*)workspace;
+    sp.labels = labels;
+    return launch_sample<true>(chosen, n_chosen, labels, ld, nullptr, nullptr, pyr_host->total, census, pos_list, pos_cap, B,
+                               max_num, pos_num, seed, seed_step, sp, *pyr_host, stream);
 }
 
 int b2d_counter_add(unsigned long long* cell, unsigned long long inc, void* stream) {
diff --git a/pytorch-faster-rcnn_b200/fused.py b/pytorch-faster-rcnn_b200/fused.py
--- a/pytorch-faster-rcnn_b200/fused.py
+++ b/pytorch-faster-rcnn_b200/fused.py
@@ -102,15 +102,20 @@
 class BatchedTargets(object):
 
     def __init__(self, B, n_boxes, gt_ld, assigner, sampler, means, stds, device, pyramid=None, border=0.0,
-                 prepend_gt=False, seed=0):
+                 prepend_gt=False, seed=0, sparse=False):
         self.B, self.N, self.gt_ld, self.pyr = B, int(n_boxes), int(gt_ld), pyramid
         self.pos_iou, self.neg_iou, self.min_pos = (np.float32(assigner[k]) for k in ("pos_iou", "neg_iou", "min_pos_iou"))
         self.max_num, self.pos_num = int(sampler["max_num"]), int(sampler["pos_num"])
         self.border, self.prepend, self.seed = float(border), int(bool(prepend_gt)), int(seed)
         self.out_ld = self.N + (self.gt_ld if prepend_gt else 0)
+        shapes = [(pyramid.c.lv[l].ws[a], pyramid.c.lv[l].hs[a]) for l in range(pyramid.c.num_levels)
+                  for a in range(pyramid.c.lv[l].A)] if pyramid is not None else []
+        self.sparse = bool(sparse) and pyramid is not None and not prepend_gt and self.gt_ld <= 4096 and \
+            min(self.pos_iou, self.neg_iou, self.min_pos) > 0 and all(w > 0 and h > 0 for w, h in shapes)
+        self._dense_from = None
         i32, f32, i64 = torch.int32, torch.float32, torch.int64
-        self.labels = torch.empty((B, self.out_ld), dtype=i64, device=device)
-        self.iou = torch.empty((B, self.out_ld), dtype=f32, device=device)
+        self._labels = torch.empty((B, self.out_ld), dtype=i64, device=device)
+        self._iou = torch.empty((B, self.out_ld), dtype=f32, device=device)
         self.census = torch.zeros((B, 4), dtype=i32, device=device)
         self.pos_list = torch.empty((B, self.out_ld), dtype=i32, device=device)
         self.colmax = torch.empty((B, self.gt_ld), dtype=i32, device=device)
@@ -132,11 +137,26 @@
     def reset_step(self):
         self.step_cell.zero_()
 
+    @property
+    def labels(self):
+        self._materialize()
+        return self._labels
+
+    @property
+    def iou(self):
+        self._materialize()
+        return self._iou
+
+    def _materialize(self):
+        if self._dense_from is not None:
+            gt, gt_count, img_hw = self._dense_from
+            self._assign_dense(gt, gt_count, None, 0, None, img_hw)
+
     def target_args(self, gt, gt_count, gt_label):
         assert self.fused
         a = _C.RoiTargetArgs()
         dp = lambda t: t.data_ptr() if t is not None else None
-        a.labels, a.max_iou, a.out_ld = dp(self.labels), dp(self.iou), self.out_ld
+        a.labels, a.max_iou, a.out_ld = dp(self._labels), dp(self._iou), self.out_ld
         a.gt, a.gt_ld, a.gt_count, a.gt_label = dp(gt), self.gt_ld, dp(gt_count), dp(gt_label)
         a.pos_iou, a.neg_iou, a.min_pos_iou = float(self.pos_iou), float(self.neg_iou), float(self.min_pos)
         a.prepend_gt, a.census, a.pos_list, a.pos_cap = self.prepend, dp(self.census), dp(self.pos_list), self.out_ld
@@ -150,7 +170,10 @@
         return a
 
     def slice(self, b0, b1):
-        return _batch_view(self, b0, b1)
+        v = _batch_view(self, b0, b1)
+        if self._dense_from is not None:
+            v._dense_from = tuple(t[b0:b1] for t in self._dense_from)
+        return v
 
     def __call__(self, gt, gt_count, gt_label=None, boxes=None, box_count=None, img_hw=None, tail_stream=None):
         pyr = ctypes.byref(self.pyr.c) if boxes is None else None
@@ -159,7 +182,7 @@
             _C.call("b2d_counter_add", _C.ptr(self.step_cell), 1, _C.stream())
         base_seed = (self.seed * 1000003 + 0x632BE59BD9B4E019 * self.b0) & 0xFFFFFFFFFFFFFFFF
         if self.fused and boxes is not None:
-            _C.call("b2d_roi_targets_fused", _C.ptr(self.labels), _C.ptr(self.iou), self.out_ld, _C.ptr(boxes), box_ld,
+            _C.call("b2d_roi_targets_fused", _C.ptr(self._labels), _C.ptr(self._iou), self.out_ld, _C.ptr(boxes), box_ld,
                     _C.ptr(box_count), self.N, _C.ptr(gt), self.gt_ld, _C.ptr(gt_count), _C.ptr(gt_label), self.B,
                     float(self.pos_iou), float(self.neg_iou), float(self.min_pos), self.prepend, _C.ptr(self.census),
                     _C.ptr(self.pos_list), self.out_ld, _C.ptr(self.chosen), _C.ptr(self.n_chosen), self.max_num,
@@ -167,29 +190,46 @@
                     _C.ptr(self.tar_box), _C.ptr(self.tar_gt), _C.ptr(self.tar_param), _C.ptr(self.tar_label),
                     _C.ptr(self.tar_is_gt), self.means, self.stds, _C.stream())
             return self
-        _C.call("b2d_assign_max_iou", _C.ptr(self.labels), _C.ptr(self.iou), self.out_ld, _C.ptr(boxes), box_ld,
-                _C.ptr(box_count), self.N, pyr, _C.ptr(img_hw), self.border, _C.ptr(gt), self.gt_ld, _C.ptr(gt_count),
-                self.B, float(self.pos_iou), float(self.neg_iou), float(self.min_pos), self.prepend,
-                _C.ptr(self.census), _C.ptr(self.pos_list), self.out_ld, _C.ptr(self.colmax), self.colmax.numel() * 4,
-                _C.stream())
+        if self.sparse:
+            self._dense_from = (gt, gt_count, img_hw)
+            _C.call("b2d_assign_sparse", _C.ptr(self.census), _C.ptr(self.pos_list), self.out_ld, pyr, _C.ptr(img_hw),
+                    self.border, _C.ptr(gt), self.gt_ld, _C.ptr(gt_count), self.B, float(self.pos_iou),
+                    float(self.neg_iou), float(self.min_pos), _C.ptr(self.colmax), self.colmax.numel() * 4, _C.stream())
+        else:
+            self._assign_dense(gt, gt_count, boxes, box_ld, box_count, img_hw)
         cnt, cnt_add = (box_count, gt_count) if (self.prepend and box_count is not None) else \
             ((None, gt_count) if self.prepend else (box_count, None))
         n = self.N if cnt is None else 0
         if tail_stream is not None:
             tail_stream.wait_stream(torch.cuda.current_stream())
             with torch.cuda.stream(tail_stream):
-                self._sample_encode(cnt, cnt_add, n, base_seed, boxes, box_ld, pyr, gt, gt_count, gt_label)
+                self._sample_encode(cnt, cnt_add, n, base_seed, boxes, box_ld, pyr, gt, gt_count, gt_label, img_hw)
             return self
-        self._sample_encode(cnt, cnt_add, n, base_seed, boxes, box_ld, pyr, gt, gt_count, gt_label)
+        self._sample_encode(cnt, cnt_add, n, base_seed, boxes, box_ld, pyr, gt, gt_count, gt_label, img_hw)
         return self
 
-    def _sample_encode(self, cnt, cnt_add, n, base_seed, boxes, box_ld, pyr, gt, gt_count, gt_label):
-        _C.call("b2d_sample_labels", _C.ptr(self.chosen), _C.ptr(self.n_chosen), _C.ptr(self.labels), self.out_ld,
-                _C.ptr(cnt), _C.ptr(cnt_add), n, _C.ptr(self.census), _C.ptr(self.pos_list), self.out_ld, self.B,
-                self.max_num, self.pos_num, base_seed, _C.ptr(self.step_cell), _C.stream())
+    def _assign_dense(self, gt, gt_count, boxes, box_ld, box_count, img_hw):
+        pyr = ctypes.byref(self.pyr.c) if boxes is None else None
+        _C.call("b2d_assign_max_iou", _C.ptr(self._labels), _C.ptr(self._iou), self.out_ld, _C.ptr(boxes), box_ld,
+                _C.ptr(box_count), self.N, pyr, _C.ptr(img_hw), self.border, _C.ptr(gt), self.gt_ld, _C.ptr(gt_count),
+                self.B, float(self.pos_iou), float(self.neg_iou), float(self.min_pos), self.prepend,
+                _C.ptr(self.census), _C.ptr(self.pos_list), self.out_ld, _C.ptr(self.colmax), self.colmax.numel() * 4,
+                _C.stream())
+
+    def _sample_encode(self, cnt, cnt_add, n, base_seed, boxes, box_ld, pyr, gt, gt_count, gt_label, img_hw):
+        if self.sparse:
+            _C.call("b2d_sample_labels_sparse", _C.ptr(self.chosen), _C.ptr(self.n_chosen), _C.ptr(self._labels),
+                    self.out_ld, _C.ptr(self.census), _C.ptr(self.pos_list), self.out_ld, pyr, _C.ptr(img_hw),
+                    self.border, _C.ptr(gt), self.gt_ld, _C.ptr(gt_count), _C.ptr(self.colmax), self.B,
+                    float(self.pos_iou), float(self.neg_iou), float(self.min_pos), self.max_num, self.pos_num, base_seed,
+                    _C.ptr(self.step_cell), _C.stream())
+        else:
+            _C.call("b2d_sample_labels", _C.ptr(self.chosen), _C.ptr(self.n_chosen), _C.ptr(self._labels), self.out_ld,
+                    _C.ptr(cnt), _C.ptr(cnt_add), n, _C.ptr(self.census), _C.ptr(self.pos_list), self.out_ld, self.B,
+                    self.max_num, self.pos_num, base_seed, _C.ptr(self.step_cell), _C.stream())
         _C.call("b2d_encode_targets", _C.ptr(self.tar_box), _C.ptr(self.tar_gt), _C.ptr(self.tar_param),
                 _C.ptr(self.tar_label), _C.ptr(self.tar_is_gt), _C.ptr(self.chosen), _C.ptr(self.n_chosen),
-                self.max_num, _C.ptr(self.labels), self.out_ld, _C.ptr(boxes), box_ld, pyr, _C.ptr(gt), self.gt_ld,
+                self.max_num, _C.ptr(self._labels), self.out_ld, _C.ptr(boxes), box_ld, pyr, _C.ptr(gt), self.gt_ld,
                 _C.ptr(gt_count), _C.ptr(gt_label), self.prepend, self.means, self.stds, self.B, _C.stream())
         return self
 
@@ -252,7 +292,7 @@
         self.pyr = AnchorPyramid(strides, grids)
         self.proposals = RpnProposals(self.pyr, B, rpn_proposal, z4, rpn_stds, device)
         self.rpn_targets = BatchedTargets(B, self.pyr.total, gt_ld, rpn_assigner, rpn_sampler, z4, rpn_stds, device,
-                                          pyramid=self.pyr, border=allowed_border, seed=seed)
+                                          pyramid=self.pyr, border=allowed_border, seed=seed, sparse=True)
         self.roi_targets = BatchedTargets(B, self.proposals.P, gt_ld, rcnn_assigner, rcnn_sampler, z4, rcnn_stds,
                                           device, prepend_gt=True, seed=seed + 1)
         self.step_cell = torch.ones(1, dtype=torch.int64, device=device)
```

Result: faster. 33220 (median of 6 runs) (+1.5%).
